# mjevans26/Satellite_ComputerVision

Hardware: AMD Instinct MI355X
Metric: tiles/sec (train) 256x256x4 U-Net (higher is better)
Workload: dtype bf16; 1 GPU; U-Net 256x256x4 bfloat16 training, batch 64 per GPU (BASELINE configs[1]); global_batch=64, parallelism=dp1, loss=weighted_categorical_crossentropy, optimizer=adam(9e-4)

## Files before the change

### include/satcv.h

```cpp
#ifndef SATCV_H
#define SATCV_H
#include <stdint.h>
#ifdef __cplusplus
extern "C" {
#endif

typedef double satcv_stat_t;

enum { SATCV_OK = 0, SATCV_ERR_INVALID = -1, SATCV_ERR_HIP = -2, SATCV_ERR_UNSUPPORTED = -3 };
enum { SATCV_F32 = 0, SATCV_BF16 = 1,
       SATCV_FP8 = 2 ,
       SATCV_FP8X = 3 ,
       SATCV_F64 = 4  };
#define SATCV_STAT_ROWS 32

const char* satcv_version(void);
const char* satcv_last_error(void);
int satcv_device_info(int32_t* out4);

int satcv_ingest_nhwc(const float* src, void* dst, int64_t npix, int32_t c, int32_t cpad,
                      int32_t dtype, void* stream);
int satcv_ingest_nhwc_scaled(const float* src, void* dst, int64_t npix, int32_t c, int32_t cpad, float mul, int32_t dtype, void* stream);
int satcv_ingest_chw(const void* src, int32_t src_kind, float scale, void* dst, int32_t n,
                     int32_t c, int32_t h, int32_t w, int32_t cpad, int32_t dtype, void* stream);

int satcv_pack_weights(const float* src, void* dst_fwd, void* dst_dgrad, int32_t kh, int32_t kw,
                       int32_t cin, int32_t cout, int32_t cin_pad, int32_t transposed,
                       int32_t dtype, void* stream);
typedef struct { const float* src; void* dst; int32_t mode, taps, cin, cout, kpad, npad; } satcv_pack_job;
int64_t satcv_pack_job_items(const satcv_pack_job* job);
int satcv_pack_weights_batched(const satcv_pack_job* jobs_dev, const int64_t* prefix_dev, int32_t njobs, int64_t total_items, int32_t dtype,
                               void* stream);

typedef struct satcv_conv_desc {
  const void* x0;
  const void* x1;
  int32_t c0, c1;
  const float* in_scale;
  const float* in_shift;
  int32_t in_relu;
  const void* w;
  const float* bias;
  void* y;
  int32_t ldy;
  satcv_stat_t* stats;
  int32_t stats_ld;
  int32_t n, h, w_;
  int32_t cout;
  int32_t cout_pad;
  int32_t kh, kw, dil;
  int32_t mode_in;
  int32_t mode_out;
  int32_t f;
  int32_t cstat;
  int32_t out_relu;
  int32_t dtype;
  int32_t accumulate;
  int32_t stride, hin, win;
  const float* out_scale;
  void* pool_y; int32_t pool_ld, pool_f;
  const void* bst_y; const void* bst_y1; int32_t bst_ld, bst_ld1, bst_split;
  const float* bst_scale; const float* bst_shift; const float* bst_mean; const float* bst_rstd; int32_t bst_relu;
  int32_t tile_policy;
  int32_t pair_n, pair_c0, pair_c1;
} satcv_conv_desc;
// ... 19 lines not shown
} satcv_wgrad_desc;
int64_t satcv_conv2d_wgrad_workspace(const satcv_wgrad_desc* d);
int satcv_conv2d_wgrad(const satcv_wgrad_desc* d, void* stream);

typedef struct satcv_reduce_job {
  const float* ws; float* dw;
  int32_t nslab, taps, kpad, npad, cin, nvalid, transposed, accumulate, lanes, pad_;
} satcv_reduce_job;
int satcv_conv2d_wgrad_reduce_job(const satcv_wgrad_desc* d, satcv_reduce_job* job);
int64_t satcv_reduce_job_items(const satcv_reduce_job* job);
int satcv_reduce_slabs_batched(const satcv_reduce_job* jobs_dev, const int64_t* prefix_dev, int32_t njobs, int64_t total_items, void* stream);

typedef struct satcv_bwdf_desc {
  const void* g; const void* yraw; int32_t ldg;
  const float* bn_scale; const float* bn_shift; const float* bn_mean; const float* bn_rstd;
  const float* bn_coef;
  int32_t linear;
  const void* x0; const void* x1; int32_t c0, c1;
  const float* in_scale; const float* in_shift; int32_t in_relu;
  const void* w_dgrad;
  void* dx; int32_t lddx;
  float* dw; int32_t cin, cout;
  int32_t n, h, w_;
  int32_t kh, kw, dil;
  float* workspace; int64_t workspace_bytes;
  int32_t dtype;
  int32_t accumulate;
  satcv_stat_t* bst_sums; int32_t bst_sums_ld;
  const float* bst_mean; const float* bst_rstd;
  int32_t bst_act_form;
  const void* dpool; int32_t lddp; const void* amax;
  const float* hg_dlogits; const float* hg_w; int32_t hg_ncls;
  int32_t defer_reduce;
} satcv_bwdf_desc;
int64_t satcv_conv2d_bwd_fused_workspace(const satcv_bwdf_desc* d);
int satcv_conv2d_bwd_fused(const satcv_bwdf_desc* d, void* stream);
int satcv_conv2d_bwd_fused_reduce_job(const satcv_bwdf_desc* d, satcv_reduce_job* job);

typedef struct satcv_ctbf_desc {
  const void* g; int32_t ldg;
  const void* yup; int32_t ldy;
  const float* bn_scale; const float* bn_shift; const float* bn_mean; const float* bn_rstd;
  const float* bn_c1; const float* bn_c2; int32_t linear;
  const void* x; int32_t ldx;
  const float* in_scale; const float* in_shift; int32_t in_relu;
  const void* w_dgrad; int32_t w_npad;
  void* dx; int32_t lddx;
  float* dw; int32_t cin, cout;
  int32_t n, h, w_, f;
  float* workspace; int64_t workspace_bytes;
  int32_t dtype, accumulate, defer_reduce;
  satcv_stat_t* bst_sums; int32_t bst_sums_ld; const float* bst_mean; const float* bst_rstd;
} satcv_ctbf_desc;
int64_t satcv_convt_bwd_fused_workspace(const satcv_ctbf_desc* d);
int satcv_convt_bwd_fused(const satcv_ctbf_desc* d, void* stream);
int satcv_convt_bwd_fused_reduce_job(const satcv_ctbf_desc* d, satcv_reduce_job* job);

int satcv_bn_finalize_train(satcv_stat_t* stats, int32_t stats_ld, int32_t c, float count,
                            const float* gamma, const float* beta, float eps, float momentum,
                            int32_t updates, int32_t bessel, float* moving_mean, float* moving_var,
                            float* scale, float* shift, float* mean, float* rstd, void* stream);
int satcv_bn_affine_infer(const float* gamma, const float* beta, const float* moving_mean,
                          const float* moving_var, float eps, int32_t c, float* scale, float* shift,
                          void* stream);
typedef struct satcv_bn_affine_job {
  const float* gamma; const float* beta; const float* moving_mean; const float* moving_var;
// ... 208 lines not shown
```

### satellite_computervision_amd/_lib.py

```python
import ctypes as C
import os

import torch

_HERE = os.path.dirname(os.path.abspath(__file__))
LIB_PATH = os.environ.get('SATCV_LIB') or os.path.join(_HERE, 'libsatcv.so')

F32, BF16, FP8, FP8X, F64 = 0, 1, 2, 3, 4
STAT_ROWS = 32
COMPOSITE_MAX_T = 256

c_i32, c_i64, c_f32, c_vp = C.c_int32, C.c_int64, C.c_float, C.c_void_p


class ConvDesc(C.Structure):
    _fields_ = [('x0', c_vp), ('x1', c_vp), ('c0', c_i32), ('c1', c_i32),
                ('in_scale', c_vp), ('in_shift', c_vp), ('in_relu', c_i32),
                ('w', c_vp), ('bias', c_vp), ('y', c_vp), ('ldy', c_i32),
                ('stats', c_vp), ('stats_ld', c_i32),
                ('n', c_i32), ('h', c_i32), ('w_', c_i32),
                ('cout', c_i32), ('cout_pad', c_i32),
                ('kh', c_i32), ('kw', c_i32), ('dil', c_i32),
                ('mode_in', c_i32), ('mode_out', c_i32), ('f', c_i32),
                ('cstat', c_i32), ('out_relu', c_i32), ('dtype', c_i32), ('accumulate', c_i32),
# ... 25 lines not shown
                ('crop_y', c_i32), ('crop_x', c_i32), ('crop_h', c_i32), ('crop_w', c_i32),
                ('origins', c_vp), ('total', c_i32), ('first', c_i32), ('dst', c_vp), ('dst_kind', c_i32),
                ('h', c_i32), ('w_', c_i32), ('ldd', c_i32), ('doff', c_i32), ('accumulate', c_i32)]


class CompositeDesc(C.Structure):
    _fields_ = [('src', c_vp), ('src_kind', c_i32), ('t', c_i32), ('c', c_i32), ('h', c_i32), ('w_', c_i32), ('offsets', c_vp),
                ('median', c_vp), ('ld_med', c_i32), ('coff_med', c_i32), ('norm', c_vp), ('ld_norm', c_i32), ('coff_norm', c_i32),
                ('use_fill', c_i32), ('fill', c_f32)]


class WgradDesc(C.Structure):
    _fields_ = [('x0', c_vp), ('x1', c_vp), ('c0', c_i32), ('c1', c_i32),
                ('in_scale', c_vp), ('in_shift', c_vp), ('in_relu', c_i32),
                ('dy', c_vp), ('lddy', c_i32), ('dw', c_vp),
                ('cin', c_i32), ('cout', c_i32),
                ('n', c_i32), ('h', c_i32), ('w_', c_i32),
                ('kh', c_i32), ('kw', c_i32), ('dil', c_i32),
                ('mode_dy', c_i32), ('f', c_i32), ('transposed', c_i32),
                ('workspace', c_vp), ('workspace_bytes', c_i64), ('dtype', c_i32), ('accumulate', c_i32), ('whole_chip', c_i32), ('defer_reduce', c_i32)]


class BwdfDesc(C.Structure):
    _fields_ = [('g', c_vp), ('yraw', c_vp), ('ldg', c_i32),
                ('bn_scale', c_vp), ('bn_shift', c_vp), ('bn_mean', c_vp), ('bn_rstd', c_vp), ('bn_coef', c_vp), ('linear', c_i32),
                ('x0', c_vp), ('x1', c_vp), ('c0', c_i32), ('c1', c_i32),
                ('in_scale', c_vp), ('in_shift', c_vp), ('in_relu', c_i32),
                ('w_dgrad', c_vp), ('dx', c_vp), ('lddx', c_i32),
                ('dw', c_vp), ('cin', c_i32), ('cout', c_i32),
                ('n', c_i32), ('h', c_i32), ('w_', c_i32), ('kh', c_i32), ('kw', c_i32), ('dil', c_i32),
                ('workspace', c_vp), ('workspace_bytes', c_i64), ('dtype', c_i32), ('accumulate', c_i32),
                ('bst_sums', c_vp), ('bst_sums_ld', c_i32), ('bst_mean', c_vp), ('bst_rstd', c_vp), ('bst_act_form', c_i32),
                ('dpool', c_vp), ('lddp', c_i32), ('amax', c_vp),
                ('hg_dlogits', c_vp), ('hg_w', c_vp), ('hg_ncls', c_i32), ('defer_reduce', c_i32)]


class CtbfDesc(C.Structure):
    _fields_ = [('g', c_vp), ('ldg', c_i32), ('yup', c_vp), ('ldy', c_i32),
                ('bn_scale', c_vp), ('bn_shift', c_vp), ('bn_mean', c_vp), ('bn_rstd', c_vp), ('bn_c1', c_vp), ('bn_c2', c_vp), ('linear', c_i32),
                ('x', c_vp), ('ldx', c_i32), ('in_scale', c_vp), ('in_shift', c_vp), ('in_relu', c_i32),
                ('w_dgrad', c_vp), ('w_npad', c_i32), ('dx', c_vp), ('lddx', c_i32), ('dw', c_vp), ('cin', c_i32), ('cout', c_i32),
                ('n', c_i32), ('h', c_i32), ('w_', c_i32), ('f', c_i32), ('workspace', c_vp), ('workspace_bytes', c_i64),
                ('dtype', c_i32), ('accumulate', c_i32), ('defer_reduce', c_i32),
                ('bst_sums', c_vp), ('bst_sums_ld', c_i32), ('bst_mean', c_vp), ('bst_rstd', c_vp)]


class ReduceJob(C.Structure):
    _fields_ = [('ws', c_vp), ('dw', c_vp), ('nslab', c_i32), ('taps', c_i32), ('kpad', c_i32), ('npad', c_i32), ('cin', c_i32), ('nvalid', c_i32),
                ('transposed', c_i32), ('accumulate', c_i32), ('lanes', c_i32), ('pad_', c_i32)]


class BnBwdDesc(C.Structure):
    _fields_ = [('da', c_vp), ('ldda', c_i32), ('dpool', c_vp), ('lddp', c_i32), ('f', c_i32),
                ('yraw', c_vp), ('ldy', c_i32),
                ('scale', c_vp), ('shift', c_vp), ('mean', c_vp), ('rstd', c_vp),
                ('sums', c_vp), ('sums_ld', c_i32), ('coef', c_vp),
                ('dy', c_vp), ('lddy_out', c_i32), ('dbias', c_vp),
                ('n', c_i32), ('h', c_i32), ('w_', c_i32), ('c', c_i32), ('dtype', c_i32), ('linear', c_i32),
                ('yraw1', c_vp), ('ldy1', c_i32), ('dy1', c_vp), ('lddy1', c_i32), ('c_split', c_i32),
                ('sk_sums', c_vp), ('sk_sums_ld', c_i32)]


class HeadDesc(C.Structure):
    _fields_ = [('x', c_vp), ('ldx', c_i32), ('cin', c_i32),
                ('in_scale', c_vp), ('in_shift', c_vp), ('w', c_vp), ('b', c_vp),
                ('ncls', c_i32), ('activation', c_i32), ('thresh', c_f32),
                ('probs', c_vp), ('classes', c_vp), ('dlogits', c_vp),
# ... 7 lines not shown
                ('c_out', c_vp), ('h_out', c_vp), ('ldh', c_i32), ('gates_out', c_vp),
                ('stats', c_vp), ('stats_ld', c_i32),
                ('dh_a', c_vp), ('lddh_a', c_i32), ('dh_b', c_vp), ('lddh_b', c_i32), ('dc_next', c_vp),
                ('dz_out', c_vp), ('lddz', c_i32), ('dc_prev_out', c_vp),
                ('npix', c_i64), ('filters', c_i32), ('rec_act', c_i32), ('act', c_i32), ('dtype', c_i32)]


class DenseSrc(C.Structure):
    _fields_ = [('x', c_vp), ('ld', c_i32), ('cin', c_i32), ('dtype', c_i32),
                ('in_scale', c_vp), ('in_shift', c_vp), ('in_relu', c_i32),
                ('hs', c_i32), ('ws', c_i32),
                ('dx', c_vp), ('lddx', c_i32), ('dx_dtype', c_i32)]


class DenseDesc(C.Structure):
    _fields_ = [('src', DenseSrc * 2), ('nsrc', c_i32),
                ('w', c_vp), ('b', c_vp), ('cout', c_i32),
                ('activation', c_i32), ('max_value', c_f32),
                ('out', c_vp), ('classes', c_vp), ('z_out', c_vp),
                ('npix', c_i64), ('h', c_i32), ('w_', c_i32),
                ('dout', c_vp), ('dz_out', c_vp), ('dw', c_vp), ('db', c_vp)]


_SIGS = {
    'satcv_version': (C.c_char_p, []),
    'satcv_last_error': (C.c_char_p, []),
    'satcv_device_info': (C.c_int, [C.POINTER(c_i32)]),
    'satcv_ingest_nhwc': (C.c_int, [c_vp, c_vp, c_i64, c_i32, c_i32, c_i32, c_vp]),
    'satcv_ingest_nhwc_scaled': (C.c_int, [c_vp, c_vp, c_i64, c_i32, c_i32, c_f32, c_i32, c_vp]),
    'satcv_ingest_chw': (C.c_int, [c_vp, c_i32, c_f32, c_vp, c_i32, c_i32, c_i32, c_i32, c_i32, c_i32, c_vp]),
    'satcv_pack_weights': (C.c_int, [c_vp, c_vp, c_vp, c_i32, c_i32, c_i32, c_i32, c_i32, c_i32, c_i32, c_vp]),
    'satcv_pack_job_items': (c_i64, [C.POINTER(PackJob)]),
    'satcv_pack_weights_batched': (C.c_int, [c_vp, c_vp, c_i32, c_i64, c_i32, c_vp]),
    'satcv_conv2d_igemm': (C.c_int, [C.POINTER(ConvDesc), c_vp]),
    'satcv_conv2d_igemm_pipelined': (C.c_int, [C.POINTER(ConvDesc)]),
    'satcv_conv2d_wgrad_workspace': (c_i64, [C.POINTER(WgradDesc)]),
    'satcv_conv2d_wgrad': (C.c_int, [C.POINTER(WgradDesc), c_vp]),
    'satcv_conv2d_wgrad_reduce_job': (C.c_int, [C.POINTER(WgradDesc), C.POINTER(ReduceJob)]),
    'satcv_reduce_job_items': (c_i64, [C.POINTER(ReduceJob)]),
    'satcv_reduce_slabs_batched': (C.c_int, [c_vp, c_vp, c_i32, c_i64, c_vp]),
    'satcv_conv2d_bwd_fused_workspace': (c_i64, [C.POINTER(BwdfDesc)]),
    'satcv_conv2d_bwd_fused': (C.c_int, [C.POINTER(BwdfDesc), c_vp]),
    'satcv_conv2d_bwd_fused_reduce_job': (C.c_int, [C.POINTER(BwdfDesc), C.POINTER(ReduceJob)]),
    'satcv_convt_bwd_fused_workspace': (c_i64, [C.POINTER(CtbfDesc)]),
    'satcv_convt_bwd_fused': (C.c_int, [C.POINTER(CtbfDesc), c_vp]),
    'satcv_convt_bwd_fused_reduce_job': (C.c_int, [C.POINTER(CtbfDesc), C.POINTER(ReduceJob)]),
    'satcv_bn_finalize_train': (C.c_int, [c_vp, c_i32, c_i32, c_f32, c_vp, c_vp, c_f32, c_f32, c_i32, c_i32,
                                          c_vp, c_vp, c_vp, c_vp, c_vp, c_vp, c_vp]),
    'satcv_bn_affine_infer': (C.c_int, [c_vp, c_vp, c_vp, c_vp, c_f32, c_i32, c_vp, c_vp, c_vp]),
    'satcv_bn_affine_infer_batched': (C.c_int, [c_vp, c_i32, c_f32, c_vp]),
    'satcv_bn_relu_pool': (C.c_int, [c_vp, c_vp, c_vp, c_vp, c_i32, c_vp, c_vp, c_i32, c_i32, c_i32, c_i32, c_i32, c_i32, c_i32, c_vp]),
    'satcv_bn_relu_pool_amax': (C.c_int, [c_vp, c_vp, c_vp, c_vp, c_i32, c_vp, c_vp, c_vp, c_i32, c_i32, c_i32, c_i32, c_i32, c_i32, c_i32, c_vp]),
    'satcv_bn_bwd_reduce': (C.c_int, [C.POINTER(BnBwdDesc), c_vp]),
    'satcv_bn_bwd_finalize': (C.c_int, [c_vp, c_i32, c_i32, c_f32, c_vp, c_vp, c_vp, c_i32, c_vp]),
    'satcv_bn_bwd_apply': (C.c_int, [C.POINTER(BnBwdDesc), c_vp]),
    'satcv_bn_bwd_finalize2': (C.c_int, [c_vp, c_i32, c_vp, c_i32, c_i32, c_f32, c_vp, c_vp, c_vp, c_vp, c_vp, c_vp, c_vp, c_i32, c_vp]),
    'satcv_maxpool': (C.c_int, [c_vp, c_vp, c_i32, c_i32, c_i32, c_i32, c_i32, c_i32, c_i32, c_i32, c_vp]),
    'satcv_affine_requant': (C.c_int, [c_vp, c_i32, c_vp, c_vp, c_i32, c_vp, c_i32, c_i64, c_i32, c_i32, c_i32, c_vp]),
    'satcv_add_act': (C.c_int, [c_vp, c_vp, c_vp, c_vp, c_vp, c_vp, c_i32, c_vp, c_i64, c_i32, c_i32, c_vp]),
    'satcv_relu_bwd': (C.c_int, [c_vp, c_vp, c_i64, c_i32, c_vp]),
    'satcv_bias_grad_workspace': (c_i64, [c_i64, c_i32]),
    'satcv_bias_grad': (C.c_int, [c_vp, c_i32, c_i64, c_i32, c_i32, c_vp, c_vp, c_vp]),
    'satcv_upsample_head': (C.c_int, [c_vp, c_i32, c_i32, c_i32, c_i32, c_i32, c_i32, c_f32, c_vp, c_vp, c_vp]),
    'satcv_dropout_mask': (C.c_int, [C.c_uint64, C.c_uint64, c_f32, c_i64, c_vp, c_vp]),
    'satcv_dropout_apply': (C.c_int, [c_vp, c_i32, c_vp, c_vp, c_i32, c_vp, c_i32, c_i32, c_vp, c_i32, c_i32, c_i32, c_i32, c_i32, c_vp]),
    'satcv_tile_channel_mean': (C.c_int, [C.POINTER(TileDesc), c_vp, c_vp]),
# ... 71 lines not shown
```

### satellite_computervision_amd/csrc/api.hip

```cpp
#include "common.hpp"
#include <cstring>
#include <cstdarg>
#include <cstdio>
#include <cstdlib>
#include <mutex>
#include <vector>

static thread_local char g_err[512] = "";
void satcv_set_error(const char* fmt, ...) {
  va_list ap;
  va_start(ap, fmt);
  vsnprintf(g_err, sizeof(g_err), fmt, ap);
  va_end(ap);
}

extern "C" const char* satcv_version(void) { return "satcv 0.1 (gfx950)"; }
extern "C" const char* satcv_last_error(void) { return g_err; }

extern "C" int satcv_device_info(int32_t* out4) {
  SATCV_CHECK(out4, "device_info: null");
  int dev = 0;
  SATCV_HIP(hipGetDevice(&dev));
  hipDeviceProp_t p;
  SATCV_HIP(hipGetDeviceProperties(&p, dev));
// ... 74 lines not shown
extern "C" int satcv_prof_enable(int32_t kind_mask) {
  g_prof_mask = kind_mask;
  return SATCV_OK;
}
extern "C" int satcv_prof_collect(int32_t kind, double* total_ms, int64_t* launches, double* flops) {
  SATCV_CHECK(kind >= 0 && kind < PROF_KINDS && total_ms && launches && flops, "prof_collect: bad args");
  std::lock_guard<std::mutex> lk(g_prof_mu);
  double ms = 0, fl = 0;
  for (auto& r : g_prof[kind]) {
    (void)hipEventSynchronize(r.b);
    float t = 0;
    if (hipEventElapsedTime(&t, r.a, r.b) == hipSuccess) ms += t;
    fl += r.flops;
    (void)hipEventDestroy(r.a); (void)hipEventDestroy(r.b);
  }
  *total_ms = ms; *launches = (int64_t)g_prof[kind].size(); *flops = fl;
  g_prof[kind].clear();
  return SATCV_OK;
}

static int env_int(const char* name, int dflt) { const char* e = getenv(name); return e ? atoi(e) : dflt; }
int g_opt_igemm_db = env_int("SATCV_DB", 1);
int g_opt_wgrad_db = env_int("SATCV_WGRAD_DB", 1);
int g_opt_igemm_sched = env_int("SATCV_IGEMM_SCHED", 0);
int g_opt_igemm_thin = env_int("SATCV_THIN", 1);
int g_opt_igemm_m16 = env_int("SATCV_M16", 1);
int g_opt_m16p = env_int("SATCV_M16P", 1);
extern int g_m16p_launches;
int g_tr_launches = 0;
int g_opt_thin_roles = env_int("SATCV_THIN_ROLES", 1);
int g_opt_m16p_prio = env_int("SATCV_M16P_PRIO", 30);
int g_opt_wgrad_m16 = env_int("SATCV_WGRAD_M16", 0);
int g_opt_splitk = env_int("SATCV_SPLITK", 0);
static int* opt_slot(const char* key) {
  if (!key) return nullptr;
  if (!strcmp(key, "igemm_db")) return &g_opt_igemm_db;
  if (!strcmp(key, "igemm_thin")) return &g_opt_igemm_thin;
  if (!strcmp(key, "wgrad_db")) return &g_opt_wgrad_db;
  if (!strcmp(key, "igemm_sched")) return &g_opt_igemm_sched;
  if (!strcmp(key, "splitk")) return &g_opt_splitk;
  if (!strcmp(key, "igemm_m16")) return &g_opt_igemm_m16;
  if (!strcmp(key, "thin_roles")) return &g_opt_thin_roles;
  if (!strcmp(key, "thin_roles_launches")) return &g_tr_launches;
  if (!strcmp(key, "m16p")) return &g_opt_m16p;
  if (!strcmp(key, "m16p_prio")) return &g_opt_m16p_prio;
  if (!strcmp(key, "wgrad_m16")) return &g_opt_wgrad_m16;
  if (!strcmp(key, "m16p_launches")) return &g_m16p_launches;
  return nullptr;
}
extern "C" int satcv_set_option(const char* key, int32_t value) {
  int* p = opt_slot(key);
  SATCV_CHECK(p, "set_option: unknown key '%s'", key ? key : "(null)");
  *p = value;
  return SATCV_OK;
}
extern int g_ws_launches;
extern "C" int satcv_get_option(const char* key, int32_t* value) {
  if (key && value && !strcmp(key, "igemm_thin_launches")) { *value = g_ws_launches; return SATCV_OK; }
  int* p = opt_slot(key);
  SATCV_CHECK(p && value, "get_option: unknown key '%s'", key ? key : "(null)");
  *value = *p;
  return SATCV_OK;
}

static uint32_t g_crc_tab[8][256];
static bool g_crc_init = [] {
  for (uint32_t i = 0; i < 256; ++i) {
    uint32_t c = i;
    for (int k = 0; k < 8; ++k) c = (c & 1) ? (c >> 1) ^ 0x82F63B78u : c >> 1;
    g_crc_tab[0][i] = c;
  }
  for (uint32_t i = 0; i < 256; ++i)
    for (int t = 1; t < 8; ++t) g_crc_tab[t][i] = (g_crc_tab[t - 1][i] >> 8) ^ g_crc_tab[0][g_crc_tab[t - 1][i] & 0xff];
  return true;
}();
extern "C" uint32_t satcv_crc32c(const void* data, uint64_t nbytes, uint32_t crc_in) {
  const unsigned char* p = reinterpret_cast<const unsigned char*>(data);
  uint32_t c = ~crc_in;
  while (nbytes >= 8) {
    uint32_t lo, hi;
// ... 10 lines not shown
```

### satellite_computervision_amd/csrc/common.hpp

```cpp
#pragma once
#include <hip/hip_runtime.h>
#include <hip/hip_fp8.h>
#include <stdint.h>
#include <type_traits>
#include "../../include/satcv.h"

typedef __bf16 bf16;
typedef __hip_fp8_e4m3 fp8;
struct fp8s : public __hip_fp8_e4m3 { using __hip_fp8_e4m3::__hip_fp8_e4m3; };
using i32x8 = __attribute__((ext_vector_type(8))) int;
using i32x4 = __attribute__((ext_vector_type(4))) int;

template <typename T> struct KTraits { static constexpr int EL = 8, SUB = 1; };
template <> struct KTraits<fp8s> { static constexpr int EL = 16, SUB = 2; };
using bf16x8 = __attribute__((ext_vector_type(8))) __bf16;
using bf16x4 = __attribute__((ext_vector_type(4))) __bf16;
using short4v = __attribute__((ext_vector_type(4))) short;
using f32x16 = __attribute__((ext_vector_type(16))) float;
using f32x4 = __attribute__((ext_vector_type(4))) float;

void satcv_set_error(const char* fmt, ...);
#define SATCV_CHECK(cond, ...)                        \
  do {                                                \
    if (!(cond)) {                                    \
// ... 196 lines not shown
    const bf16x8 v = __builtin_bit_cast(bf16x8, r.q[0]);
#pragma unroll
    for (int i = 0; i < 8; ++i) out[i] = (float)v[i];
  } else if constexpr (std::is_same<T, float>::value) {
    const float* f = reinterpret_cast<const float*>(&r.q[0]);
#pragma unroll
    for (int i = 0; i < 8; ++i) out[i] = f[i];
  } else {
    const fp8* b = reinterpret_cast<const fp8*>(&r.q);
#pragma unroll
    for (int i = 0; i < 8; ++i) out[i] = (float)b[i];
  }
}
template <typename T>
__device__ __forceinline__ void keep8(const Raw8<T>& r) {
  if constexpr (std::is_same<T, fp8>::value) { asm volatile("" :: "v"(r.q.x), "v"(r.q.y)); }
  else {
#pragma unroll
    for (int i = 0; i < Raw8<T>::NQ; ++i) asm volatile("" :: "v"(r.q[i].x), "v"(r.q[i].y), "v"(r.q[i].z), "v"(r.q[i].w));
  }
}
template <typename T>
__device__ __forceinline__ Raw8<T> select8(bool keep, const Raw8<T>& r) {
  Raw8<T> o;
  if constexpr (std::is_same<T, fp8>::value) {
    o.q = make_uint2(keep ? r.q.x : 0u, keep ? r.q.y : 0u);
  } else {
#pragma unroll
    for (int i = 0; i < Raw8<T>::NQ; ++i) o.q[i] = make_uint4(keep ? r.q[i].x : 0u, keep ? r.q[i].y : 0u, keep ? r.q[i].z : 0u, keep ? r.q[i].w : 0u);
  }
  return o;
}

template <typename T>
__device__ __forceinline__ float round_to(float x) {
  if constexpr (std::is_same<T, bf16>::value) return (float)(bf16)x;
  else if constexpr (std::is_same<T, fp8>::value) return (float)(fp8)x;
  else return x;
}

__device__ __forceinline__ float wave_sum(float v) {
#pragma unroll
  for (int o = 32; o > 0; o >>= 1) v += __shfl_xor(v, o, 64);
  return v;
}

typedef __attribute__((address_space(3))) char satcv_lds_char;
__device__ __forceinline__ unsigned lds_addr_of(const void* p) { return (unsigned)(uintptr_t)(satcv_lds_char*)p; }
__device__ __forceinline__ void lds_dma16(const void* gbase, unsigned voff, unsigned lds_dst) {
  unsigned keep;
  asm volatile("s_mov_b32 %0, m0\n\ts_mov_b32 m0, %3\n\ts_nop 0\n\tglobal_load_lds_dwordx4 %2, %1\n\ts_mov_b32 m0, %0"
               : "=&s"(keep) : "s"(gbase), "v"(voff), "s"(lds_dst) : "memory");
}
__device__ __forceinline__ void dma_wait_all() { asm volatile("s_waitcnt vmcnt(0)" ::: "memory"); }

#define SATCV_STAT_REPL 32
```

### satellite_computervision_amd/csrc/conv_bwd_fused.hip

```cpp
#include "igemm_common.hpp"
#include <cstdlib>
#include <cstring>

#ifndef BWDF_ABL
#define BWDF_ABL 0
#endif
#define FABL(bit) ((BWDF_ABL & (bit)) != 0)

int wgrad_reduce_slabs(const float* ws, float* dw, int nslab, int taps, int kpad, int npad, int cin, int nvalid, int accumulate, hipStream_t st);
void reduce_job_fill(satcv_reduce_job* job, const float* ws, float* dw, int nslab, int taps, int kpad, int npad, int cin, int nvalid, int transposed, int accumulate);
void satcv_prof_begin(int kind, double flops, hipStream_t st);
void satcv_prof_end(int kind, hipStream_t st);

struct BwdfArgs {
  IgemmArgs e;
  const void* g; const void* yraw; int ldg;
  const float* bn_scale; const float* bn_shift; const float* bn_mean; const float* bn_rstd; const float* bn_coef; int bn_c, linear;
  const void* x0; const void* x1; int c0, c1;
  const float* in_scale; const float* in_shift; int in_relu;
  const void* w;
  float* ws;
  int tiles_x, tiles_y;
  satcv_stat_t* bst_sums; int bst_ld; const float* bst_mean; const float* bst_rstd;
  int bst_act_form;
  const void* dp; int lddp; const unsigned char* amax;
  const float* hg_dl; const float* hg_w;
};

__device__ __forceinline__ bf16x4 tr_read4(const bf16* p) {
  short4v v = __builtin_amdgcn_ds_read_tr16_b64_v4i16((__attribute__((address_space(3))) short4v*)(p));
  return __builtin_bit_cast(bf16x4, v);
}

template <int CIN, int COUT, int NW, int WPS, bool POOL = false, bool NODG = false, int CINS = CIN, bool HG = false>
__global__ __launch_bounds__(NW * 64, WPS) void bwd_fused_kernel(const BwdfArgs a, const int total_tiles) {
  static_assert(!HG || !POOL, "the head feeds a decoder block");
  typedef bf16 T;
  constexpr int TW = 32, TH = 8, BM = 256, RL = TH + 2, CL = TW + 2, PITCH = CL, EL = 8, NTHREADS = NW * 64;
  constexpr int SD = COUT / 8, SX = CIN / 8, SXR = CINS / 8;
  constexpr int DSTRIDE = RL * PITCH * EL;
  constexpr int XSTRIDE = BM * EL + 32;
  static_assert((DSTRIDE * 2) % 256 == 64 && (XSTRIDE * 2) % 256 == 64, "plane strides must be 64 B modulo 256 B");
  constexpr int D_ITEMS = RL * CL * SD, DI = (D_ITEMS + NTHREADS - 1) / NTHREADS;
  constexpr int X_ITEMS = BM * SXR, XI = X_ITEMS / NTHREADS;
  static_assert(X_ITEMS % NTHREADS == 0 && NTHREADS % SD == 0 && NTHREADS % SXR == 0, "item -> thread mapping");
  constexpr int XPIX_STEP = NTHREADS / SXR;
  static_assert(XPIX_STEP % 32 == 0, "x items of a thread must share a column");
  constexpr int MT = 8 / NW, NT = CIN / 32;
#ifdef BWDF_NOBAL
  constexpr int NTILE = (CIN / 32) * (COUT / 32) * 9, FULL = (NTILE + NW - 1) / NW, REM = 0, WT = FULL;
#else
  constexpr int NTILE = (CIN / 32) * (COUT / 32) * 9, FULL = NTILE / NW, REM = NTILE % NW, WT = FULL + (REM ? 1 : 0);
#endif
  constexpr bool GUARD = FULL * NW > NTILE;
  constexpr int WPP = REM ? NW / REM : 1, KPW = REM ? 16 / WPP : 0;
  static_assert(REM == 0 || (NW % REM == 0 && 16 % WPP == 0 && KPW % 2 == 0), "left-over products must split evenly along K");
  constexpr int W_ITEMS = NODG ? 0 : 9 * SD * CIN;
  constexpr size_t R0_BYTES = ((size_t)(SD * DSTRIDE + SX * XSTRIDE) * sizeof(T) + 127) / 128 * 128;
  constexpr size_t W_BYTES = (size_t)W_ITEMS * EL * sizeof(T);
  constexpr size_t O_BYTES = (size_t)BM * (CIN + 8) * sizeof(T);
  constexpr bool O_ALIAS = O_BYTES <= (size_t)SD * DSTRIDE * sizeof(T);
  constexpr size_t TAB_BYTES = (size_t)(SD * 32 + SX * 16 + (HG ? 2 * COUT : 0)) * sizeof(float);
  static_assert(!NODG || O_ALIAS || true, "");
  constexpr size_t O_OFF = O_ALIAS ? 0 : (R0_BYTES + W_BYTES + TAB_BYTES + 127) / 128 * 128;
  extern __shared__ __attribute__((aligned(16))) unsigned char smem_raw[];
  T* ldsD = reinterpret_cast<T*>(smem_raw);
  T* ldsX = ldsD + SD * DSTRIDE;
  T* ldsW = reinterpret_cast<T*>(smem_raw + R0_BYTES);
  float* tabD = reinterpret_cast<float*>(smem_raw + R0_BYTES + W_BYTES);
// ... 12 lines not shown
    const float sc = a.bn_scale[ch], sh = a.bn_shift[ch], mu = a.bn_mean[ch], rs = a.bn_rstd[ch], c1 = a.bn_coef[ch], c2 = a.bn_coef[a.bn_c + ch];
    float* t = tabD + (ch >> 3) * 32 + (ch & 7);
    t[0] = sc; t[8] = sh; t[16] = -sc * c2 * rs; t[24] = sc * (c2 * rs * mu - c1);
  }
  if constexpr (HG) {
    for (int ch = tid; ch < COUT; ch += NTHREADS) {
      float* t = tabH + (ch >> 3) * 16 + (ch & 7);
      t[0] = a.hg_w[ch * 2]; t[8] = a.hg_w[ch * 2 + 1];
    }
  }
  for (int ch = tid; ch < CINS; ch += NTHREADS) {
    float* t = tabX + (ch >> 3) * 16 + (ch & 7);
    t[0] = a.in_scale ? a.in_scale[ch] : 1.f; t[8] = a.in_scale ? a.in_shift[ch] : 0.f;
  }
  const float lin_lo = a.linear ? -INFINITY : 0.f;
  const bool xaff = a.in_scale != nullptr;
  const unsigned xrelu_lim = a.in_relu != 0 ? 0u : 0x80008000u;

  const int slot_d = tid % SD, slot_x = tid % SXR;
  constexpr int DPK = (DI + 2) / 3;
  unsigned d_pk[DPK];
#pragma unroll
  for (int k = 0; k < DPK; ++k) d_pk[k] = 0;
#pragma unroll
  for (int j = 0; j < DI; ++j) {
    const int it = tid + j * NTHREADS;
    const int p = it / SD, c = p % CL, L = p / CL;
    d_pk[j / 3] |= (unsigned)(it < D_ITEMS ? (L << 6) | c : 0x3ff) << (10 * (j % 3));
  }
  auto d_item = [&](int j) -> int { return (int)((d_pk[j / 3] >> (10 * (j % 3))) & 0x3ffu); };
  const int g_rowstride = a.e.w_ * a.ldg;
  const unsigned gy_lane = (unsigned)slot_d * EL;
  const int xch0 = slot_x * EL;
  const bool xsecond = xch0 >= a.c0;
  const T* xsrc = xsecond ? reinterpret_cast<const T*>(a.x1) + (xch0 - a.c0) : reinterpret_cast<const T*>(a.x0) + xch0;
  const int xcs = xsecond ? a.c1 : a.c0;
  const int xq0 = tid / SXR;
  const int x_l0 = slot_x * XSTRIDE + xq0 * EL;
  const int x_eoff0 = ((xq0 / TW) * a.e.w_ + (xq0 % TW)) * xcs, x_estep = (XPIX_STEP / TW) * a.e.w_ * xcs;

  int a_off[MT];
#pragma unroll
  for (int m = 0; m < MT; ++m) {
    const int q = (wave * MT + m) * 32 + r;
    a_off[m] = ((q / TW) * PITCH + (q % TW)) * EL;
  }
  const int gi = lane >> 4, i16 = lane & 15;
  const int chb = 16 * (gi & 1) + 4 * (i16 & 3);
  const int pk = 8 * (gi >> 1) + (i16 >> 2);
  const int tr_x = (chb >> 3) * XSTRIDE + pk * EL + (chb & 7);
  const int tr_d = (chb >> 3) * DSTRIDE + pk * EL + (chb & 7);

  auto tile_origin = [&](int v, int& n0, int& y0, int& x0) {
    const int tx = v % a.tiles_x; v /= a.tiles_x;
    const int ty = v % a.tiles_y;
    n0 = v / a.tiles_y; y0 = ty * TH; x0 = tx * TW;
  };
  auto next_origin = [&](int& n0, int& y0, int& x0) {
    x0 += TW;
    if (x0 >= a.e.w_) { x0 = 0; y0 += TH; if (y0 >= a.e.h) { y0 = 0; ++n0; } }
  };
  Raw8<T> rg[HG ? 1 : DI], ry[DI], rx[XI];
  float2 rdl[HG ? DI : 1];
  Raw8<T> rp[POOL ? DI : 1];
  uint2 ra[POOL ? DI : 1];
  const int hp = a.e.h >> 1, wpool = a.e.w_ >> 1;
  unsigned valid = 0;
  auto issue_loads = [&](int n0, int y0, int x0) -> unsigned {
    unsigned vm = 0;
// ... 110 lines not shown
          }
        }
        Raw8<T> v;
        if constexpr (FABL(2) && !HG) { v = rg[j]; v.q[0].x ^= ry[j].q[0].x; }
        else {
          bf16x8 o;
#pragma unroll
          for (int e = 0; e < 8; ++e) {
            const float act = yv[e] * prm[e] + prm[8 + e];
            const float gm = act > lin_lo ? gv[e] : 0.f;
            o[e] = (bf16)(prm[e] * gm + (prm[16 + e] * yv[e] + prm[24 + e]));
          }
          v.q[0] = __builtin_bit_cast(uint4, o);
        }
        v = select8<T>((valid >> j) & 1u, v);
        const int pk_ = d_item(j);
        if (pk_ != 0x3ff) lstore8<T>(ldsD + slot_d * DSTRIDE + __mul24((pk_ >> 6) * CL + (pk_ & 63), EL), v);
        __builtin_amdgcn_sched_barrier(0);
      }
    }
    {
      float sc[8], sh[8];
      if (xaff) {
        int toff = slot_x * 16;
        asm volatile("" : "+v"(toff));
        const float4* tp = reinterpret_cast<const float4*>(tabX + toff);
        const float4 s0 = tp[0], s1 = tp[1], h0 = tp[2], h1 = tp[3];
        sc[0] = s0.x; sc[1] = s0.y; sc[2] = s0.z; sc[3] = s0.w; sc[4] = s1.x; sc[5] = s1.y; sc[6] = s1.z; sc[7] = s1.w;
        sh[0] = h0.x; sh[1] = h0.y; sh[2] = h0.z; sh[3] = h0.w; sh[4] = h1.x; sh[5] = h1.y; sh[6] = h1.z; sh[7] = h1.w;
      }
#pragma unroll
      for (int j = 0; j < XI; ++j) {
        Raw8<T> v = rx[j];
        if (xaff) v = affine8_lim(v, sc, sh, xrelu_lim);
        lstore8<T>(ldsX + x_l0 + j * (XPIX_STEP * EL), v);
      }
    }
    __syncthreads();
    const int tn0 = n0, ty0 = y0, tx0 = x0;
    if (t + 1 < t_hi) { next_origin(n0, y0, x0); valid = issue_loads(n0, y0, x0); }

#pragma unroll
    for (int tt = 0; tt < FULL; ++tt) {
      if (!FABL(8) && (!GUARD || tt < FULL - 1 || __builtin_amdgcn_readfirstlane(wave) + (FULL - 1) * NW < NTILE)) {
        const T* xa = ldsX + w_xo[tt] + tr_x;
        const T* da = ldsD + w_do[tt] + tr_d;
        bf16x4 fa[2][2], fb[2][2];
        auto read_k = [&](const T* xp, const T* dp, int u, int buf) {
          const int xq = u * 16 * EL, dq = ((u >> 1) * PITCH + (u & 1) * 16) * EL;
          fa[buf][0] = tr_read4(xp + xq); fa[buf][1] = tr_read4(xp + xq + 4 * EL);
          fb[buf][0] = tr_read4(dp + dq); fb[buf][1] = tr_read4(dp + dq + 4 * EL);
        };
        read_k(xa, da, 0, 0);
#pragma unroll 1
        for (int grp = 0; grp < TH / 2; ++grp) {
          const T* xp = xa + grp * (64 * EL);
          const T* dp = da + grp * (2 * PITCH * EL);
          const int wrap = grp + 1 < TH / 2 ? 1 : 1 - TH / 2;
#pragma unroll
          for (int u = 0; u < 4; ++u) {
            asm volatile("" ::: "memory");
            if (u < 3) read_k(xp, dp, u + 1, (u + 1) & 1);
            else read_k(xp + wrap * (64 * EL), dp + wrap * (2 * PITCH * EL), 0, 0);
            __builtin_amdgcn_sched_barrier(0);
            const bf16x8 afr = __builtin_shufflevector(fa[u & 1][0], fa[u & 1][1], 0, 1, 2, 3, 4, 5, 6, 7);
            const bf16x8 bfr = __builtin_shufflevector(fb[u & 1][0], fb[u & 1][1], 0, 1, 2, 3, 4, 5, 6, 7);
// ... 148 lines not shown
      atomicAdd(rowp + a.bst_ld + tid, (satcv_stat_t)s2);
    }
  }
}

template <int CIN, int COUT, int NW, bool NODG = false>
struct BwdfGeom {
  static constexpr int SD = COUT / 8, SX = CIN / 8;
  static constexpr size_t R0 = ((size_t)(SD * (10 * 34 * 8) + SX * (256 * 8 + 32)) * 2 + 127) / 128 * 128;
  static constexpr size_t O_BYTES = (size_t)256 * (CIN + 8) * 2;
  static constexpr bool O_ALIAS = O_BYTES <= (size_t)SD * (10 * 34 * 8) * 2;
  static constexpr size_t BASE = R0 + (NODG ? 0 : (size_t)9 * SD * CIN * 16) + (size_t)(SD * 32 + SX * 16 + 2 * COUT) * 4;
  static constexpr size_t LDS0 = O_ALIAS ? BASE : (BASE + 127) / 128 * 128 + O_BYTES;
  static constexpr size_t RED = (size_t)16 * NW * 64 * 4;
  static constexpr size_t LDS = LDS0 > RED ? LDS0 : RED;
};

static int g_ncu = 0;
static int bwdf_grid(size_t lds, int waves, int wps, long long total) {
  if (!g_ncu) {
    int dev = 0; hipDeviceProp_t p;
    if (hipGetDevice(&dev) != hipSuccess || hipGetDeviceProperties(&p, dev) != hipSuccess) return -1;
    g_ncu = p.multiProcessorCount;
  }
  int per_cu = (int)((160 * 1024) / lds);
  const int by_waves = 4 * wps / waves;
  if (per_cu > by_waves) per_cu = by_waves;
  if (per_cu < 1) per_cu = 1;
  long long grid = (long long)g_ncu * per_cu;
  if (grid > total) grid = total;
  return (int)grid;
}

static bool bwdf_shape_ok(const satcv_bwdf_desc* d, int& cin_s) {
  cin_s = d->c0 + d->c1;
  if (d->dtype != SATCV_BF16 || d->kh != 3 || d->kw != 3 || d->dil != 1) return false;
  if (d->x1 && d->c0 % 8 != 0) return false;
  if (d->h % 8 != 0 || d->w_ % 32 != 0) return false;
  if (d->ldg % 8 != 0 || ((uintptr_t)d->g % 16) != 0 || ((uintptr_t)d->yraw % 16) != 0) return false;
  if (d->hg_dlogits && (!d->hg_w || d->hg_ncls != 2 || d->dpool || ((uintptr_t)d->hg_dlogits % 8) != 0)) return false;
  if (d->dx && (d->lddx % 8 != 0 || ((uintptr_t)d->dx % 16) != 0)) return false;
  if ((long long)d->w_ * d->ldg >= (1 << 23)) return false;
  if (d->dpool) {
    if (!d->amax || d->lddp % 8 != 0 || ((uintptr_t)d->dpool % 16) != 0 || ((uintptr_t)d->amax % 8) != 0 || d->x1) return false;
    if (d->dx) return cin_s == 32 && d->cin == 32 && d->cout == 64;
    return cin_s == 16 && d->cin <= 16 && d->cout == 32 && !d->bst_sums;
  }
  if (!d->dx) return false;
  if (d->bst_sums && cin_s == 64 && d->cout == 64) return false;
  if (!((cin_s == 32 && d->cout == 32) || (cin_s == 64 && d->cout == 32) || (cin_s == 64 && d->cout == 64))) return false;
  if (d->cin != cin_s) return false;
  return true;
}

template <int CIN, int COUT, int NW, int WPS, bool POOL = false, bool NODG = false, int CINS = CIN, bool HG = false>
static int bwdf_launch(const satcv_bwdf_desc* d, hipStream_t st, bool query, int64_t* ws_bytes, satcv_reduce_job* job = nullptr) {
  using G = BwdfGeom<CIN, COUT, NW, NODG>;
  static_assert(G::LDS <= 160 * 1024, "tile + weights exceed the LDS");
  const long long total = (long long)d->n * (d->h / 8) * (d->w_ / 32);
  const int grid = bwdf_grid(G::LDS, NW, WPS, total);
  if (grid <= 0) { satcv_set_error("bwd_fused: device query failed"); return SATCV_ERR_HIP; }
  const size_t need = (size_t)grid * 9 * CIN * COUT * sizeof(float);
  if (job) { reduce_job_fill(job, d->workspace, d->dw, grid, 9, CIN, COUT, d->cin, COUT, 0, d->accumulate); return SATCV_OK; }
  if (query) { *ws_bytes = (int64_t)need; return SATCV_OK; }
  SATCV_CHECK((size_t)d->workspace_bytes >= need, "bwd_fused: workspace %lld < %zu", (long long)d->workspace_bytes, need);
  BwdfArgs a;
  memset(&a, 0, sizeof(a));
  a.e.y = d->dx; a.e.ldy = d->lddx; a.e.n = d->n; a.e.h = d->h; a.e.w_ = d->w_; a.e.cout = CIN; a.e.cout_pad = CIN; a.e.cstat = CIN;
  a.e.imgs = 1; a.e.rpi = 8; a.e.tiles_x = d->w_ / 32; a.e.tiles_y = d->h / 8; a.e.n_tiles = 1;
  a.g = d->g; a.yraw = d->yraw; a.ldg = d->ldg;
  a.bn_scale = d->bn_scale; a.bn_shift = d->bn_shift; a.bn_mean = d->bn_mean; a.bn_rstd = d->bn_rstd; a.bn_coef = d->bn_coef; a.bn_c = d->cout; a.linear = d->linear;
  a.x0 = d->x0; a.x1 = d->x1; a.c0 = d->c0; a.c1 = d->c1; a.in_scale = d->in_scale; a.in_shift = d->in_shift; a.in_relu = d->in_relu;
  a.w = d->w_dgrad; a.ws = d->workspace; a.tiles_x = d->w_ / 32; a.tiles_y = d->h / 8;
  a.bst_sums = d->bst_sums; a.bst_ld = d->bst_sums_ld; a.bst_mean = d->bst_mean; a.bst_rstd = d->bst_rstd; a.bst_act_form = d->bst_act_form;
  a.dp = d->dpool; a.lddp = d->lddp; a.amax = reinterpret_cast<const unsigned char*>(d->amax);
  a.hg_dl = d->hg_dlogits; a.hg_w = d->hg_w;
  auto kern = bwd_fused_kernel<CIN, COUT, NW, WPS, POOL, NODG, CINS, HG>;
  { const int rc = satcv_ensure_dynamic_lds(reinterpret_cast<const void*>(kern), G::LDS); if (rc) return rc; }
  const double flops = (NODG ? 2.0 : 4.0) * d->n * d->h * d->w_ * (double)CINS * COUT * 9;
  satcv_prof_begin(3, flops, st);
  hipLaunchKernelGGL(kern, dim3(grid), dim3(NW * 64), G::LDS, st, a, (int)total);
  satcv_prof_end(3, st);
  hipError_t e = hipGetLastError();
  if (e != hipSuccess) { satcv_set_error("bwd_fused launch: %s", hipGetErrorString(e)); return SATCV_ERR_HIP; }
  if (d->defer_reduce) return SATCV_OK;
  return wgrad_reduce_slabs(d->workspace, d->dw, grid, 9, CIN, COUT, d->cin, COUT, d->accumulate, st);
}

static int bwdf_dispatch(const satcv_bwdf_desc* d, hipStream_t st, bool query, int64_t* ws_bytes, satcv_reduce_job* job = nullptr) {
  int cin_s;
  if (!bwdf_shape_ok(d, cin_s)) return SATCV_ERR_UNSUPPORTED;
  if (d->dpool) {
    if (d->dx) return bwdf_launch<32, 64, 4, 1, true, false>(d, st, query, ws_bytes, job);
    return bwdf_launch<32, 32, 8, 2, true, true, 16>(d, st, query, ws_bytes, job);
  }
  if (cin_s == 32 && d->hg_dlogits) return bwdf_launch<32, 32, 8, 2, false, false, 32, true>(d, st, query, ws_bytes, job);
  if (d->hg_dlogits) return SATCV_ERR_UNSUPPORTED;
  if (cin_s == 32) return bwdf_launch<32, 32, 8, 2>(d, st, query, ws_bytes, job);
  if (d->cout == 32) return bwdf_launch<64, 32, 8, 2>(d, st, query, ws_bytes, job);
  return bwdf_launch<64, 64, 4, 1>(d, st, query, ws_bytes, job);
}

extern "C" int satcv_conv2d_bwd_fused_reduce_job(const satcv_bwdf_desc* d, satcv_reduce_job* job) {
  SATCV_CHECK(d && job && d->dw && d->workspace, "bwd_fused_reduce_job: null pointer");
  return bwdf_dispatch(d, nullptr, false, nullptr, job);
}

extern "C" int64_t satcv_conv2d_bwd_fused_workspace(const satcv_bwdf_desc* d) {
  int64_t nb = -1;
  if (!d || bwdf_dispatch(d, nullptr, true, &nb) != SATCV_OK) return -1;
  return nb;
}

extern "C" int satcv_conv2d_bwd_fused(const satcv_bwdf_desc* d, void* stream) {
  SATCV_CHECK(d && (d->g || d->hg_dlogits) && d->yraw && d->x0 && d->dw && d->workspace && (d->dx == nullptr || d->w_dgrad), "bwd_fused: null pointer");
  SATCV_CHECK(d->bn_scale && d->bn_shift && d->bn_mean && d->bn_rstd && d->bn_coef, "bwd_fused: BatchNorm coefficients missing");
  SATCV_CHECK((d->c1 == 0) == (d->x1 == nullptr) && d->n > 0 && d->h > 0 && d->w_ > 0, "bwd_fused: bad dims");
  SATCV_CHECK(!d->bst_sums || (d->bst_sums_ld >= d->c0 + d->c1 && (d->bst_act_form ? d->in_scale == nullptr
                               : (d->in_scale && d->in_shift && d->in_relu && d->bst_mean && d->bst_rstd))),
              "bwd_fused: the fused sums need the input's BatchNorm (in_scale / in_shift with ReLU, bst_mean / bst_rstd), or an activated input with bst_act_form");
  const int rc = bwdf_dispatch(d, reinterpret_cast<hipStream_t>(stream), false, nullptr);
  if (rc == SATCV_ERR_UNSUPPORTED) satcv_set_error("bwd_fused: shape outside the kernel's limits (ask satcv_conv2d_bwd_fused_workspace first)");
  return rc;
}
```

### satellite_computervision_amd/csrc/conv_igemm.hip

```cpp
#include "igemm_common.hpp"
#include <cstdlib>

template <typename T, int TW, int WM, int WN, int MT, int NT, int KS>
__global__ __launch_bounds__(WM* WN * 64) void igemm_kernel(const IgemmArgs a) {
  constexpr int NTHREADS = WM * WN * 64;
  constexpr int BM = WM * MT * 32;
  constexpr int BN = WN * NT * 32;
  constexpr int TH = BM / TW;
  constexpr int KC = KS * 16;
  constexpr int SLOTS = KC / 8;
  extern __shared__ __attribute__((aligned(16))) unsigned char smem_raw[];
  T* ldsA = reinterpret_cast<T*>(smem_raw);
  const int a_elems = SLOTS * a.rl * a.pitch * 8;
  T* ldsB = ldsA + a_elems;

  const int tid = threadIdx.x;
  const int lane = tid & 63;
  const int wave = tid >> 6;
  const int wm = wave / WN, wn = wave % WN;
  const int r = lane & 31, hh = lane >> 5;

  int bid = blockIdx.x;
  const int nt = bid % a.n_tiles;
  int mt = bid / a.n_tiles;
// ... 208 lines not shown
template <typename T, int TW>
static int launch_tw(IgemmArgs& a, hipStream_t st) {
  const int cin = a.c0 + a.c1;
  const int nspace = a.mode_out ? a.cstat : a.cout;
  const bool ks2 = (cin % 32 == 0) && (!a.x1 || a.c0 % 32 == 0) && (a.mode_in != 1 || a.c0 % 32 == 0) &&
                   (a.kh * a.kw == 1);
  int rc = SATCV_ERR_UNSUPPORTED;
  if (nspace >= 128 && nspace % 128 == 0)
    rc = ks2 ? launch_cfg<T, TW, 2, 2, 2, 2, 2>(a, st) : launch_cfg<T, TW, 2, 2, 2, 2, 1>(a, st);
  if (rc == SATCV_ERR_UNSUPPORTED && nspace >= 64 && nspace % 64 == 0)
    rc = ks2 ? launch_cfg<T, TW, 2, 2, 2, 1, 2>(a, st) : launch_cfg<T, TW, 2, 2, 2, 1, 1>(a, st);
  if (rc == SATCV_ERR_UNSUPPORTED)
    rc = ks2 ? launch_cfg<T, TW, 4, 1, 2, 1, 2>(a, st) : launch_cfg<T, TW, 4, 1, 2, 1, 1>(a, st);
  if (rc == SATCV_ERR_UNSUPPORTED)
    rc = launch_cfg<T, TW, 2, 1, 2, 1, 1>(a, st);
  if (rc == SATCV_ERR_UNSUPPORTED) satcv_set_error("igemm: no tile configuration fits the LDS for this shape");
  return rc;
}

template <typename T>
static int launch_t(IgemmArgs& a, hipStream_t st) {
  switch (igemm_pick_tw(a.w_)) {
    case 32: return launch_tw<T, 32>(a, st);
    case 16: return launch_tw<T, 16>(a, st);
    default: return launch_tw<T, 8>(a, st);
  }
}

void satcv_prof_begin(int kind, double flops, hipStream_t st);
void satcv_prof_end(int kind, hipStream_t st);

static int igemm_fill_args(const satcv_conv_desc* d, IgemmArgs& a) {
  SATCV_CHECK(d && d->x0 && d->w && d->y, "igemm: null pointer");
  SATCV_CHECK(d->c0 > 0 && d->c0 % 16 == 0 && d->c1 % 16 == 0, "igemm: channels must be multiples of 16 (c0=%d c1=%d)", d->c0, d->c1);
  SATCV_CHECK(d->dtype != SATCV_FP8X || (d->c0 % 64 == 0 && d->c1 % 64 == 0 && !d->in_scale), "igemm: the scaled fp8 path needs channels %% 64 == 0 and no input transform");
  SATCV_CHECK((d->c1 == 0) == (d->x1 == nullptr), "igemm: x1/c1 mismatch");
  SATCV_CHECK(d->kh >= 1 && d->kw >= 1 && (d->kh & 1) && (d->kw & 1) && d->dil >= 1, "igemm: bad taps");
  SATCV_CHECK(d->n > 0 && d->h > 0 && d->w_ > 0 && d->cout > 0, "igemm: bad dims");
  SATCV_CHECK(satcv_pixels_ok(d->n, d->h, d->w_, d->f) && d->cout <= (1 << 20) && d->c0 <= (1 << 20) && d->c1 <= (1 << 20) &&
              d->kh <= 15 && d->kw <= 15 && d->dil <= (1 << 15) && d->f <= 16 && d->stride <= 16,
              "igemm: extents out of range (n*h*w must stay below 2^31 pixels, channels below 2^20)");
  SATCV_CHECK(d->cstat > 0, "igemm: cstat");
  SATCV_CHECK((!d->mode_in && !d->mode_out) || (d->f >= 2 && d->kh == 1 && d->kw == 1), "igemm: s2d/d2s need 1x1 taps and f>=2");
  SATCV_CHECK(!(d->accumulate && d->stats), "igemm: accumulate with statistics");
  SATCV_CHECK(!(d->mode_in && d->in_scale), "igemm: s2d source cannot carry an input transform");
  a.x0 = d->x0; a.x1 = d->x1; a.c0 = d->c0; a.c1 = d->c1;
  a.in_scale = d->in_scale; a.in_shift = d->in_shift; a.in_relu = d->in_relu;
  a.w = d->w; a.bias = d->bias; a.out_scale = d->out_scale; a.y = d->y; a.ldy = d->ldy;
  a.pool_y = d->pool_y; a.pool_ld = d->pool_ld; a.pool_f = d->pool_f;
  SATCV_CHECK(!d->pool_y || (d->pool_f >= 2 && !d->mode_out && !d->accumulate && d->h % d->pool_f == 0 && d->w_ % d->pool_f == 0 && d->pool_ld >= d->cout &&
                             d->cout % (d->dtype == SATCV_F32 ? 4 : (d->dtype == SATCV_BF16 ? 8 : 16)) == 0),
              "igemm: fused max-pool needs pool_f >= 2 dividing h and w_, plain output mode, whole 16-byte channel vectors");
  a.stats = d->stats; a.stats_ld = d->stats_ld;
  a.n = d->n; a.h = d->h; a.w_ = d->w_;
  a.hs = d->mode_in ? d->h * d->f : d->h; a.ws = d->mode_in ? d->w_ * d->f : d->w_;
  a.cout = d->cout; a.cout_pad = d->cout_pad;
  a.kh = d->kh; a.kw = d->kw; a.dil = d->dil;
  a.mode_in = d->mode_in; a.mode_out = d->mode_out; a.f = d->f;
  a.cstat = d->cstat; a.out_relu = d->out_relu; a.accumulate = d->accumulate;
  a.stride = d->stride > 1 ? d->stride : 1;
  if (a.stride > 1) {
    SATCV_CHECK(!d->mode_in && !d->mode_out && d->hin > 0 && d->win > 0 && d->h == (d->hin - 1) / a.stride + 1 && d->w_ == (d->win - 1) / a.stride + 1,
                "igemm: strided conv needs hin/win with h=(hin-1)/stride+1");
    a.hs = d->hin; a.ws = d->win;
  }
  a.dbg = 0;
  a.ksplit = 1; a.kslab = nullptr;
  a.bst_y = d->bst_y; a.bst_y1 = d->bst_y1; a.bst_ld = d->bst_ld; a.bst_ld1 = d->bst_ld1; a.bst_split = d->bst_y1 ? d->bst_split : 0;
  a.bst_scale = d->bst_scale; a.bst_shift = d->bst_shift; a.bst_mean = d->bst_mean; a.bst_rstd = d->bst_rstd; a.bst_relu = d->bst_relu;
  a.tile_policy = d->tile_policy;
  a.pair_n = d->pair_n; a.pair_c0 = d->pair_c0; a.pair_c1 = d->pair_c1;
  if (d->pair_n || d->pair_c0 || d->pair_c1) {
    const int epv = d->dtype == SATCV_F32 ? 4 : (d->dtype == SATCV_BF16 ? 8 : 16);
    SATCV_CHECK(d->pair_n > 0 && d->n == 2 * d->pair_n, "igemm: pair store needs n == 2 * pair_n (n=%d pair_n=%d)", d->n, d->pair_n);
    SATCV_CHECK(!d->mode_out && !d->accumulate && !d->stats && !d->bst_y, "igemm: pair store needs a plain store (no mode_out / accumulate / stats / bst_y)");
    SATCV_CHECK(d->pair_c0 >= 0 && d->pair_c1 >= 0 && d->pair_c0 + d->cout <= d->ldy && d->pair_c1 + d->cout <= d->ldy,
                "igemm: pair channel offsets %d / %d + cout %d exceed ldy %d", d->pair_c0, d->pair_c1, d->cout, d->ldy);
    SATCV_CHECK(d->pair_c0 % epv == 0 && d->pair_c1 % epv == 0, "igemm: pair channel offsets must be multiples of %d", epv);
  }
  if (d->bst_y) {
    SATCV_CHECK(d->stats && d->bst_scale && d->bst_shift && d->bst_mean && d->bst_rstd, "igemm: bst_y needs stats and the four BatchNorm vectors");
    SATCV_CHECK(!d->accumulate && !d->mode_out && !d->out_relu && !d->pool_y && d->cstat == d->cout, "igemm: bst_y needs a plain, non-accumulating store");
    SATCV_CHECK(d->bst_ld >= (d->bst_y1 ? d->bst_split : d->cout) && (!d->bst_y1 || (d->bst_split > 0 && d->bst_split < d->cout && d->bst_ld1 >= d->cout - d->bst_split)),
                "igemm: bst_y channel strides");
  }
  if (a.mode_in == 1) {
    SATCV_CHECK(!d->x1, "igemm: s2d with dual source");
    a.c1 = a.c0 * (d->f * d->f - 1);
  }
  return SATCV_OK;
}

static bool igemm_force_generic() {
  static const bool v = [] { const char* e = getenv("SATCV_IGEMM"); return e && e[0] == 'g'; }();
  return v;
}

extern "C" int satcv_conv2d_igemm_pipelined(const satcv_conv_desc* d) {
  IgemmArgs a;
  if (!d || igemm_fill_args(d, a) != SATCV_OK || igemm_force_generic()) return 0;
  if (a.kh == 3 && a.kw == 3 && a.stride == 1 && a.dil >= a.h && a.dil >= a.w_) { a.kh = a.kw = 1; a.dil = 1; }
  if (d->bst_y && a.dil == 3) {
    IgemmArgs b = a;
    b.bst_y = nullptr; b.bst_y1 = nullptr;
    if (igemm_ws_launch(b, d->dtype, nullptr, true) == SATCV_OK) return 0;
  }
  return igemm_fast_launch(a, d->dtype, nullptr, true) == SATCV_OK ? 1 : 0;
}

extern "C" int satcv_conv2d_igemm(const satcv_conv_desc* d, void* stream) {
  IgemmArgs a;
  int rc = igemm_fill_args(d, a);
  if (rc) return rc;
  hipStream_t st = reinterpret_cast<hipStream_t>(stream);
  const double flops = 2.0 * d->n * d->h * d->w_ * (double)d->cout * (double)(a.c0 + a.c1) * d->kh * d->kw;
  if (a.kh == 3 && a.kw == 3 && a.stride == 1 && a.dil >= a.h && a.dil >= a.w_) {
    const size_t esz = d->dtype == SATCV_BF16 ? 2 : 4;
    a.w = reinterpret_cast<const unsigned char*>(a.w) + (size_t)4 * ((a.c0 + a.c1) / 8) * a.cout_pad * 8 * esz;
    a.kh = a.kw = 1; a.dil = 1;
  }
  satcv_prof_begin(d->kh * d->kw > 1 ? 0 : 1, flops, st);
  rc = SATCV_ERR_UNSUPPORTED;
  if (!igemm_force_generic()) {
    rc = convt_thin_launch(a, d->dtype, st);
    if (rc == SATCV_ERR_UNSUPPORTED) rc = convt_thin_dgrad_launch(a, d->dtype, st);
    if (rc == SATCV_ERR_UNSUPPORTED) rc = igemm_tr_launch(a, d->dtype, st, false);
    if (rc == SATCV_ERR_UNSUPPORTED) rc = igemm_ws_launch(a, d->dtype, st, false);
    if (rc == SATCV_ERR_UNSUPPORTED) rc = igemm_fast_launch(a, d->dtype, st);
  }
  if (rc != SATCV_ERR_UNSUPPORTED) {  }
  else if (d->dtype == SATCV_FP8 || d->dtype == SATCV_FP8X) { satcv_set_error("igemm: this fp8 shape is outside the pipelined kernel's limits"); rc = SATCV_ERR_UNSUPPORTED; }
  else if (d->out_scale || d->pool_y || d->bst_y || d->pair_n) { satcv_set_error("igemm: out_scale / pool_y / bst_y / pair store need the pipelined kernel"); rc = SATCV_ERR_UNSUPPORTED; }
  else if (d->dtype == SATCV_BF16) rc = launch_t<bf16>(a, st);
  else if (d->dtype == SATCV_F32) rc = launch_t<float>(a, st);
  else { satcv_set_error("igemm: bad dtype %d", d->dtype); rc = SATCV_ERR_INVALID; }
  satcv_prof_end(d->kh * d->kw > 1 ? 0 : 1, st);
  return rc;
}
```

### satellite_computervision_amd/csrc/conv_igemm_ws.hip

```cpp
#include "igemm_common.hpp"
#include <cstdlib>
extern int g_opt_igemm_thin;
int g_ws_launches = 0;

#ifndef SATCV_ABLATE
#define SATCV_ABLATE 0
#endif
#define WABL(bit) ((SATCV_ABLATE & (bit)) != 0)
#ifdef SATCV_STAMP
__device__ unsigned long long g_stamp_ws[8][8][8];
extern "C" int satcv_debug_read_stamps_ws(unsigned long long* out) { return hipMemcpyFromSymbol(out, HIP_SYMBOL(g_stamp_ws), sizeof(g_stamp_ws)) == hipSuccess ? 0 : -1; }
#define STAMP(t) do { __builtin_amdgcn_sched_barrier(0); asm volatile("s_memtime %0\n\ts_waitcnt lgkmcnt(0)" : "=s"(t) :: "memory"); __builtin_amdgcn_sched_barrier(0); } while (0)
#define STAMP_V(t) do { __builtin_amdgcn_sched_barrier(0); asm volatile("s_waitcnt vmcnt(0)\n\ts_memtime %0\n\ts_waitcnt lgkmcnt(0)" : "=s"(t) :: "memory"); __builtin_amdgcn_sched_barrier(0); } while (0)
#endif

template <typename T, int CIN, int NT, int WPS, int WN = 1, int DIL = 1>
__global__ __launch_bounds__(256 * WN, WPS) void igemm_ws_kernel(const IgemmArgs a, const int total_tiles) {
  constexpr int TW = 32, TH = 8, WM = 4, MT = 2, BM = 256, BN = WN * NT * 32, NTHREADS = 256 * WN, EL = 8;
  constexpr int SLOTS = CIN / EL, CL = TW + 2 * DIL, PITCH = CL, RL = TH + 2 * DIL;
  constexpr int PLANE = RL * PITCH * EL;
  constexpr int WANT = (SLOTS >= 8 ? 16 : 128 / SLOTS) / (int)sizeof(T), BANKSPAN = 128 / (int)sizeof(T);
  constexpr int SPAD = ((WANT - PLANE % BANKSPAN) % BANKSPAN + BANKSPAN) % BANKSPAN;
  constexpr int SLOT_STRIDE = PLANE + SPAD;
  constexpr int A_ITEMS = RL * CL * SLOTS, AI = (A_ITEMS + NTHREADS - 1) / NTHREADS;
  constexpr int W_ITEMS = 9 * SLOTS * BN;
  constexpr int OPITCH = BN + 16 / (int)sizeof(T);
  constexpr size_t A_BYTES = (size_t)SLOTS * SLOT_STRIDE * sizeof(T);
  constexpr size_t O_BYTES = (size_t)BM * OPITCH * sizeof(T) + (size_t)(WM + 1) * 2 * BN * sizeof(float);
  constexpr size_t R0_BYTES = ((A_BYTES > O_BYTES ? A_BYTES : O_BYTES) + 127) / 128 * 128;
  extern __shared__ __attribute__((aligned(16))) unsigned char smem_raw[];
  T* ldsA = reinterpret_cast<T*>(smem_raw);
  T* ldsW = reinterpret_cast<T*>(smem_raw + R0_BYTES);

  const int tid = threadIdx.x, lane = tid & 63, wave = tid >> 6;
  const int wm = wave / WN, wn = wave % WN;
  const int r = lane & 31, hh = lane >> 5;
  const int slot_t = tid % SLOTS;
  const T* wp = reinterpret_cast<const T*>(a.w);

  for (int it = tid; it < W_ITEMS; it += NTHREADS) {
    const int co = it % BN, run = it / BN;
    const Raw8<T> v = gload8<T>(wp + ((size_t)run * a.cout_pad + co) * EL);
    lstore8<T>(ldsW + (size_t)it * EL, v);
  }
  const int ch0 = slot_t * EL;
  const bool second = ch0 >= a.c0;
  const T* src = second ? reinterpret_cast<const T*>(a.x1) + (ch0 - a.c0) : reinterpret_cast<const T*>(a.x0) + ch0;
  const int cs = second ? a.c1 : a.c0;
  float sc[8], sh[8];
#pragma unroll
  for (int e = 0; e < 8; ++e) { sc[e] = a.in_scale ? a.in_scale[ch0 + e] : 1.f; sh[e] = a.in_scale ? a.in_shift[ch0 + e] : 0.f; }
  const bool aff = a.in_scale != nullptr;
  const unsigned relu_lim = a.in_relu != 0 ? 0u : 0x80008000u;

  int a_l[AI], a_yx[AI], a_eoff[AI];
#pragma unroll
  for (int j = 0; j < AI; ++j) {
    const int it = tid + j * NTHREADS;
    const int pix = it / SLOTS, c = pix % CL, L = pix / CL;
    a_l[j] = it < A_ITEMS ? slot_t * SLOT_STRIDE + (L * PITCH + c) * EL : -1;
    a_yx[j] = ((L - DIL) << 16) | ((c - DIL) & 0xffff);
    a_eoff[j] = ((L - DIL) * a.w_ + (c - DIL)) * cs;
  }
  int a_off[MT];
#pragma unroll
  for (int m = 0; m < MT; ++m) {
    const int q = (wm * MT + m) * 32 + r;
    a_off[m] = ((q / TW) * PITCH + (q % TW)) * EL;
  }

  auto tile_origin = [&](int v, int& n0, int& y0, int& x0) {
    const int tx = v % a.tiles_x; v /= a.tiles_x;
    const int ty = v % a.tiles_y;
    n0 = v / a.tiles_y; y0 = ty * TH; x0 = tx * TW;
  };
  auto next_origin = [&](int& n0, int& y0, int& x0) {
    x0 += TW;
    if (x0 >= a.w_) { x0 = 0; y0 += TH; if (y0 >= a.h) { y0 = 0; ++n0; } }
  };
  Raw8<T> ra[AI];
  unsigned valid = 0;
  auto issue_loads = [&](int n0, int y0, int x0) -> unsigned {
    unsigned vm = 0;
    const int ylo = -y0, yhi = a.h - y0, xlo = -x0, xhi = a.w_ - x0;
    const T* base = src + ((size_t)(n0 * a.h + y0) * a.w_ + x0) * cs;
#pragma unroll
    for (int j = 0; j < AI; ++j) {
      const int dy = a_yx[j] >> 16, dx = (int)(short)(a_yx[j] & 0xffff);
      const bool ok = a_l[j] >= 0 && dy >= ylo && dy < yhi && dx >= xlo && dx < xhi;
      vm |= (ok ? 1u : 0u) << j;
      int off = ok ? a_eoff[j] : 0;
      asm volatile("" : "+v"(off));
      if (!WABL(4)) ra[j] = gload8<T>(base + off);
      else ra[j] = zero8<T>();
    }
    return vm;
  };

  const int G = gridDim.x;
  const int xcd = blockIdx.x & 7, nx = G >> 3, remx = G & 7;
  const int bid = (xcd < remx ? xcd * (nx + 1) : remx * (nx + 1) + (xcd - remx) * nx) + (blockIdx.x >> 3);
  const int per = total_tiles / G, extra = total_tiles % G;
  const int t_lo = bid * per + (bid < extra ? bid : extra), t_hi = t_lo + per + (bid < extra ? 1 : 0);

  double carry[2] = {0.0, 0.0};
  int n0, y0, x0;
  if (t_lo < t_hi) { tile_origin(t_lo, n0, y0, x0); valid = issue_loads(n0, y0, x0); }
  __syncthreads();
#ifdef SATCV_STAMP
  unsigned long long q0, q1, q2, q3, q4, q5, q6, q7, q8, z[8] = {0, 0, 0, 0, 0, 0, 0, 0};
#endif
  for (int t = t_lo; t < t_hi; ++t) {
#ifdef SATCV_STAMP
    STAMP(q0);
    STAMP_V(q1);
#endif
#pragma unroll
    for (int j = 0; j < AI; ++j) {
      Raw8<T> v = ra[j];
      if (aff) { if constexpr (std::is_same<T, bf16>::value) v = affine8_lim(v, sc, sh, relu_lim); else v = affine8<T>(v, sc, sh, a.in_relu); }
      v = select8<T>((valid >> j) & 1u, v);
      if (a_l[j] >= 0) lstore8<T>(ldsA + a_l[j], v);
    }
#ifdef SATCV_STAMP
    STAMP(q2);
#endif
    __syncthreads();
#ifdef SATCV_STAMP
    STAMP(q3);
#endif
    const int tn0 = n0, ty0 = y0, tx0 = x0;
    if (t + 1 < t_hi) { next_origin(n0, y0, x0); valid = issue_loads(n0, y0, x0); }
#ifdef SATCV_STAMP
    STAMP(q4);
#endif
    f32x16 acc[MT][NT];
#pragma unroll
    for (int m = 0; m < MT; ++m)
#pragma unroll
      for (int n = 0; n < NT; ++n)
#pragma unroll
        for (int i = 0; i < 16; ++i) acc[m][n][i] = 0.f;
    {
      constexpr int KS = CIN / 16, STEPS = 9 * KS;
      FragT<T> af[2][MT], bf[2][NT];
      auto read_step = [&](int st, int buf) {
        const int tap = st / KS, ks = st % KS;
        const int tap_off = ((tap / 3) * DIL * PITCH + (tap % 3) * DIL) * EL;
        const int slot = ks * 2 + hh;
#pragma unroll
        for (int m = 0; m < MT; ++m) af[buf][m] = lds_frag<T>(ldsA + slot * SLOT_STRIDE + a_off[m] + tap_off);
#pragma unroll
// ... 9 lines not shown
        for (int m = 0; m < MT; ++m)
#pragma unroll
          for (int n = 0; n < NT; ++n) { if (!WABL(2)) mma32<T>(acc[m][n], af[st & 1][m], bf[st & 1][n]); }
      }
    }
#ifdef SATCV_STAMP
    STAMP(q5);
#endif
    __syncthreads();
#ifdef SATCV_STAMP
    STAMP(q6);
#endif
    igemm_epilogue<T, TW, WM, WN, MT, NT, WABL(1), true, false, false, DIL == 1>(a, acc, tn0, ty0, tx0, 0, smem_raw, carry);
#ifdef SATCV_STAMP
    STAMP(q7);
#endif
    __syncthreads();
#ifdef SATCV_STAMP
    STAMP(q8);
    z[0] += q1 - q0; z[1] += q2 - q1; z[2] += q3 - q2; z[3] += q4 - q3; z[4] += q5 - q4; z[5] += q6 - q5; z[6] += q7 - q6; z[7] += q8 - q7;
#endif
  }
  if (a.stats && tid < BN && tid < a.cout && t_lo < t_hi) {
    satcv_stat_t* rowp = a.stats + (size_t)(blockIdx.x % SATCV_STAT_ROWS) * 2 * a.stats_ld;
    atomicAdd(rowp + tid, (satcv_stat_t)carry[0]);
    atomicAdd(rowp + a.stats_ld + tid, (satcv_stat_t)carry[1]);
  }
#ifdef SATCV_STAMP
  if (blockIdx.x < 8 && lane == 0)
    for (int i = 0; i < 8; ++i) g_stamp_ws[blockIdx.x][wave][i] = z[i] / (unsigned long long)max(t_hi - t_lo, 1);
#endif
}

template <typename T, int CIN, int NT, int WPS, int WN = 1, int DIL = 1>
static int ws_cfg(IgemmArgs& a, hipStream_t st, bool dry) {
  constexpr int TW = 32, TH = 8, BN = WN * NT * 32, SLOTS = CIN / 8, RL = TH + 2 * DIL, PITCH = TW + 2 * DIL;
  constexpr int ES = (int)sizeof(T);
  constexpr int PLANE = RL * PITCH * 8;
  constexpr int WANT = (SLOTS >= 8 ? 16 : 128 / SLOTS) / ES, BANKSPAN = 128 / ES;
  constexpr int SPAD = ((WANT - PLANE % BANKSPAN) % BANKSPAN + BANKSPAN) % BANKSPAN;
  constexpr size_t A_BYTES = (size_t)SLOTS * (PLANE + SPAD) * ES;
  constexpr size_t O_BYTES = (size_t)256 * (BN + 16 / ES) * ES + (size_t)5 * 2 * BN * 4;
  constexpr size_t R0 = ((A_BYTES > O_BYTES ? A_BYTES : O_BYTES) + 127) / 128 * 128;
  constexpr size_t LDS = R0 + (size_t)9 * SLOTS * BN * 8 * ES;
  static_assert(LDS <= 160 * 1024, "weights + tile exceed the LDS");
  a.halh = a.halw = DIL;
  a.tiles_x = cdiv(a.w_, TW); a.tiles_y = cdiv(a.h, TH);
  a.rpi = TH; a.imgs = 1; a.ngroups = a.n; a.seg = RL; a.rl = RL; a.cl = PITCH; a.pitch = PITCH; a.n_tiles = 1;
  const long long total = (long long)a.n * a.tiles_y * a.tiles_x;
  if (total <= 0 || total > 0x7fffffffLL) return SATCV_ERR_UNSUPPORTED;
  if (dry) return SATCV_OK;
  auto kern = igemm_ws_kernel<T, CIN, NT, WPS, WN, DIL>;
  { const int rc = satcv_ensure_dynamic_lds(reinterpret_cast<const void*>(kern), LDS); if (rc) return rc; }
  static int ncu = 0;
  if (!ncu) {
    int dev = 0; hipDeviceProp_t p;
    if (hipGetDevice(&dev) != hipSuccess || hipGetDeviceProperties(&p, dev) != hipSuccess) { satcv_set_error("ws: device query failed"); return SATCV_ERR_HIP; }
    ncu = p.multiProcessorCount;
  }
  int per_cu = (int)((160 * 1024) / LDS);
  if (per_cu > WPS) per_cu = WPS;
  if (per_cu < 1) per_cu = 1;
  long long grid = (long long)ncu * per_cu;
  if (grid > total) grid = total;
  hipLaunchKernelGGL(kern, dim3((unsigned)grid), dim3(256 * WN), LDS, st, a, (int)total);
  ++g_ws_launches;
  hipError_t e = hipGetLastError();
  if (e != hipSuccess) { satcv_set_error("igemm_ws launch: %s", hipGetErrorString(e)); return SATCV_ERR_HIP; }
  return SATCV_OK;
}

int igemm_ws_launch(IgemmArgs& a, int dtype, hipStream_t st, bool dry) {
  if (!g_opt_igemm_thin || (dtype != SATCV_BF16 && dtype != SATCV_FP8)) return SATCV_ERR_UNSUPPORTED;
  const int cin = a.c0 + a.c1;
  if (a.kh != 3 || a.kw != 3 || (a.dil != 1 && a.dil != 3) || a.stride != 1 || a.mode_in || a.mode_out || a.bst_y) return SATCV_ERR_UNSUPPORTED;
  if (a.accumulate && (a.accumulate != 1 || dtype != SATCV_BF16 || a.stats || a.pool_y || a.out_relu || a.out_scale)) return SATCV_ERR_UNSUPPORTED;
  if (a.pool_y && (8 % a.pool_f != 0 || 32 % a.pool_f != 0)) return SATCV_ERR_UNSUPPORTED;
  if (a.dil == 3) {
    if (dtype != SATCV_BF16 || a.pool_y || a.pair_n || !(cin == 16 || cin == 32) || !(a.cout == 16 || a.cout == 32) || a.cout_pad != 32 || a.cstat != a.cout) return SATCV_ERR_UNSUPPORTED;
    if (a.x1 && (a.c0 % 8 != 0)) return SATCV_ERR_UNSUPPORTED;
    if (a.h % 8 != 0 || a.w_ % 32 != 0 || a.ldy % 8 != 0 || ((uintptr_t)a.y % 16) != 0) return SATCV_ERR_UNSUPPORTED;
    return cin == 16 ? ws_cfg<bf16, 16, 1, 2, 1, 3>(a, st, dry) : ws_cfg<bf16, 32, 1, 2, 1, 3>(a, st, dry);
  }
  if (a.cout == 16 && dtype == SATCV_BF16 && !a.pool_y && (cin == 16 || cin == 32) && a.cout_pad == 32 && a.cstat == 16 && !(a.x1 && (a.c0 % 8 != 0)) &&
      a.h % 8 == 0 && a.w_ % 32 == 0 && a.ldy % 8 == 0 && ((uintptr_t)a.y % 16) == 0) {
    return cin == 16 ? ws_cfg<bf16, 16, 1, 3>(a, st, dry) : ws_cfg<bf16, 32, 1, 3>(a, st, dry);
  }
  if (!(cin == 16 || cin == 32 || cin == 64) || !(a.cout == 32 || a.cout == 64) || a.cout_pad != a.cout || a.cstat != a.cout) return SATCV_ERR_UNSUPPORTED;
  if (a.x1 && (a.c0 % 8 != 0)) return SATCV_ERR_UNSUPPORTED;
  const int epv = dtype == SATCV_FP8 ? 16 : 8;
  if (a.h % 8 != 0 || a.w_ % 32 != 0 || a.ldy % epv != 0 || ((uintptr_t)a.y % 16) != 0) return SATCV_ERR_UNSUPPORTED;
  if (dtype == SATCV_FP8) {
    if (a.stats || cin == 16 || (a.pool_y && a.pool_ld % 16 != 0)) return SATCV_ERR_UNSUPPORTED;
    if (a.cout == 32) return cin == 32 ? ws_cfg<fp8, 32, 1, 3>(a, st, dry) : ws_cfg<fp8, 64, 1, 2>(a, st, dry);
    return cin == 32 ? ws_cfg<fp8, 32, 2, 2>(a, st, dry) : ws_cfg<fp8, 64, 1, 1, 2>(a, st, dry);
  }
  if (a.cout == 32) {
    if (cin == 16) return ws_cfg<bf16, 16, 1, 3>(a, st, dry);
    if (cin == 32) return ws_cfg<bf16, 32, 1, 3>(a, st, dry);
    return ws_cfg<bf16, 64, 1, 2>(a, st, dry);
  }
  if (cin == 16) return ws_cfg<bf16, 16, 2, 2>(a, st, dry);
  if (cin == 32) return ws_cfg<bf16, 32, 2, 2>(a, st, dry);
  return ws_cfg<bf16, 64, 1, 1, 2>(a, st, dry);
}
```

### satellite_computervision_amd/csrc/elementwise.hip

```cpp
#include "common.hpp"
#include <cstdlib>

#define EW_BLOCK 256
static inline int ew_grid(long long items, int cap = 0) {
  static const int dflt = [] { const char* e = getenv("SATCV_EW_PER_CU"); const int v = e ? atoi(e) : 6; return 256 * (v >= 1 ? v : 6); }();
  if (cap <= 0) cap = dflt;
  long long b = (items + EW_BLOCK - 1) / EW_BLOCK;
  if (b < 1) b = 1;
  if (b > cap) b = cap;
  return (int)b;
}
#define LAUNCH_OK(name)                                                          \
  do {                                                                           \
    hipError_t e__ = hipGetLastError();                                          \
    if (e__ != hipSuccess) {                                                     \
      satcv_set_error(name " launch: %s", hipGetErrorString(e__));               \
      return SATCV_ERR_HIP;                                                      \
    }                                                                            \
  } while (0)
#define DISPATCH_T(dtype, ...)                                                   \
  do {                                                                           \
    if ((dtype) == SATCV_BF16) { using T = bf16; __VA_ARGS__; }                  \
    else if ((dtype) == SATCV_F32) { using T = float; __VA_ARGS__; }             \
    else { satcv_set_error("bad dtype %d", (int)(dtype)); return SATCV_ERR_INVALID; } \
// ... 65 lines not shown
static inline int rup(int a, int b) { return (a + b - 1) / b * b; }

template <typename T, int EL = 8>
__global__ void pack_kernel(const float* __restrict__ src, T* __restrict__ dst, int mode, int taps, int cin, int cout, int kpad, int npad) {
  const int ptaps = (mode >= 2) ? 1 : taps;
  const long long total = (long long)ptaps * (kpad / EL) * npad;
  for (long long it = blockIdx.x * (long long)blockDim.x + threadIdx.x; it < total; it += (long long)gridDim.x * blockDim.x) {
    const int nn = (int)(it % npad);
    const int k8 = (int)((it / npad) % (kpad / EL));
    const int tap = (int)(it / ((long long)npad * (kpad / EL)));
    float v[EL];
#pragma unroll
    for (int e = 0; e < EL; ++e) {
      const int k = k8 * EL + e;
      float x = 0.f;
      if (mode == 0) { if (k < cin && nn < cout) x = src[((size_t)tap * cin + k) * cout + nn]; }
      else if (mode == 1) { if (k < cout && nn < cin) x = src[((size_t)(taps - 1 - tap) * cin + nn) * cout + k]; }
      else if (mode == 2) { if (k < cin && nn < taps * cout) x = src[(size_t)nn * cin + k]; }
      else { if (k < taps * cout && nn < cin) x = src[(size_t)k * cin + nn]; }
      v[e] = x;
    }
    if constexpr (EL == 8) {
      store8<T>(dst + it * 8, v);
    } else {
      float lo[8], hi[8];
#pragma unroll
      for (int e = 0; e < 8; ++e) { lo[e] = v[e]; hi[e] = v[8 + e]; }
      store8<T>(dst + it * 16, lo);
      store8<T>(dst + it * 16 + 8, hi);
    }
  }
}
template <typename T>
__global__ __launch_bounds__(EW_BLOCK) void pack_batched_kernel(const satcv_pack_job* __restrict__ jobs, const long long* __restrict__ prefix, int njobs, long long total) {
  for (long long g0 = (long long)blockIdx.x * EW_BLOCK; g0 < total; g0 += (long long)gridDim.x * EW_BLOCK) {
    int lo = 0, hi = njobs - 1;
    while (lo < hi) { const int mid = (lo + hi + 1) >> 1; if (prefix[mid] <= g0) lo = mid; else hi = mid - 1; }
    lo = __builtin_amdgcn_readfirstlane(lo);
    const satcv_pack_job j = jobs[lo];
    long long it = g0 - prefix[lo] + threadIdx.x;
    const long long real = (long long)(j.mode >= 2 ? 1 : j.taps) * (j.kpad / 8) * j.npad;
    if (it >= real) continue;
    if (j.mode == 1 && (j.kpad / 8) % 4 == 0 && j.npad % 16 == 0) {
      const int nb = j.npad / 16, kb = (j.kpad / 8) / 4;
      const int l = (int)(it % 64); long long t = it / 64;
      const int nblk = (int)(t % nb); t /= nb;
      const int kblk = (int)(t % kb); const long long tap_ = t / kb;
      const int k8_ = kblk * 4 + (l & 3), nn_ = nblk * 16 + (l >> 2);
      it = (tap_ * (j.kpad / 8) + k8_) * j.npad + nn_;
    }
    const int nn = (int)(it % j.npad);
    const int k8 = (int)((it / j.npad) % (j.kpad / 8));
    const int tap = (int)(it / ((long long)j.npad * (j.kpad / 8)));
    float v[8];
#pragma unroll
    for (int e = 0; e < 8; ++e) {
      const int k = k8 * 8 + e;
      float x = 0.f;
      if (j.mode == 0) { if (k < j.cin && nn < j.cout) x = j.src[((size_t)tap * j.cin + k) * j.cout + nn]; }
      else if (j.mode == 1) { if (k < j.cout && nn < j.cin) x = j.src[((size_t)(j.taps - 1 - tap) * j.cin + nn) * j.cout + k]; }
      else if (j.mode == 2) { if (k < j.cin && nn < j.taps * j.cout) x = j.src[(size_t)nn * j.cin + k]; }
      else { if (k < j.taps * j.cout && nn < j.cin) x = j.src[(size_t)k * j.cin + nn]; }
      v[e] = x;
    }
    store8<T>(reinterpret_cast<T*>(j.dst) + it * 8, v);
  }
}
extern "C" int64_t satcv_pack_job_items(const satcv_pack_job* j) {
  if (!j || j->kpad <= 0 || j->kpad % 8 || j->npad <= 0 || j->mode < 0 || j->mode > 3) return -1;
  const int64_t real = (int64_t)(j->mode >= 2 ? 1 : j->taps) * (j->kpad / 8) * j->npad;
  return (real + EW_BLOCK - 1) / EW_BLOCK * EW_BLOCK;
}
extern "C" int satcv_pack_weights_batched(const satcv_pack_job* jobs_dev, const int64_t* prefix_dev, int32_t njobs, int64_t total_items, int32_t dtype,
                                          void* stream) {
  SATCV_CHECK(jobs_dev && prefix_dev && njobs > 0 && total_items > 0, "pack_weights_batched: bad args");
  SATCV_CHECK(total_items % EW_BLOCK == 0, "pack_weights_batched: the prefix table must be built from satcv_pack_job_items (multiples of 256)");
  DISPATCH_T8(dtype, hipLaunchKernelGGL(pack_batched_kernel<T>, dim3(ew_grid(total_items)), dim3(EW_BLOCK), 0, (hipStream_t)stream, jobs_dev,
                                        (const long long*)prefix_dev, njobs, (long long)total_items));
  LAUNCH_OK("pack_weights_batched");
  return SATCV_OK;
}

extern "C" int satcv_pack_weights(const float* src, void* dst_fwd, void* dst_dgrad, int32_t kh, int32_t kw, int32_t cin, int32_t cout, int32_t cin_pad, int32_t transposed, int32_t dtype, void* stream) {
  SATCV_CHECK(src && cin > 0 && cout > 0 && cin_pad >= cin && cin_pad % 16 == 0, "pack_weights: bad args");
  const int taps = kh * kw;
  hipStream_t st = (hipStream_t)stream;
  if (dtype == SATCV_FP8X) {
    SATCV_CHECK(dst_fwd && !dst_dgrad && cin_pad % 16 == 0, "pack_weights: the scaled fp8 image is forward-only, cin_pad %% 16 == 0");
    const int kp = cin_pad, np = rup(transposed ? taps * cout : cout, 32);
    const long long items = (long long)(transposed ? 1 : taps) * (kp / 16) * np;
    hipLaunchKernelGGL((pack_kernel<fp8, 16>), dim3(ew_grid(items)), dim3(EW_BLOCK), 0, st, src, (fp8*)dst_fwd, transposed ? 2 : 0, taps, cin, cout, kp, np);
    LAUNCH_OK("pack_weights");
    return SATCV_OK;
  }
  DISPATCH_T8(dtype, {
    if (!transposed) {
      if (dst_fwd) { const int kp = cin_pad, np = rup(cout, 32);
        hipLaunchKernelGGL(pack_kernel<T>, dim3(ew_grid((long long)taps * (kp / 8) * np)), dim3(EW_BLOCK), 0, st, src, (T*)dst_fwd, 0, taps, cin, cout, kp, np); }
      if (dst_dgrad) { const int kp = rup(cout, 16), np = rup(cin, 32);
        hipLaunchKernelGGL(pack_kernel<T>, dim3(ew_grid((long long)taps * (kp / 8) * np)), dim3(EW_BLOCK), 0, st, src, (T*)dst_dgrad, 1, taps, cin, cout, kp, np); }
    } else {
      if (dst_fwd) { const int kp = cin_pad, np = rup(taps * cout, 32);
        hipLaunchKernelGGL(pack_kernel<T>, dim3(ew_grid((long long)(kp / 8) * np)), dim3(EW_BLOCK), 0, st, src, (T*)dst_fwd, 2, taps, cin, cout, kp, np); }
      if (dst_dgrad) { const int kp = rup(taps * cout, 16), np = rup(cin, 32);
        hipLaunchKernelGGL(pack_kernel<T>, dim3(ew_grid((long long)(kp / 8) * np)), dim3(EW_BLOCK), 0, st, src, (T*)dst_dgrad, 3, taps, cin, cout, kp, np); }
    }
  });
  LAUNCH_OK("pack_weights");
  return SATCV_OK;
}

__global__ void bn_finalize_train_kernel(satcv_stat_t* stats, int ld, int c, float count, const float* gamma, const float* beta,
                                         float eps, float momentum, int updates, int bessel, float* mm, float* mv,
// ... 1440 lines not shown
  const long long n4 = n / 4;
  for (long long i = blockIdx.x * (long long)blockDim.x + threadIdx.x; i < n4; i += (long long)gridDim.x * blockDim.x) {
    float4 pp = reinterpret_cast<float4*>(p)[i];
    const float4 gg = reinterpret_cast<const float4*>(g)[i];
    float4 mm = reinterpret_cast<float4*>(m)[i];
    float4 vv = reinterpret_cast<float4*>(v)[i];
    float4 lm = lr_mul ? reinterpret_cast<const float4*>(lr_mul)[i] : make_float4(1.f, 1.f, 1.f, 1.f);
    float* P = &pp.x; const float* Gp = &gg.x; float* M = &mm.x; float* V = &vv.x; const float* L = &lm.x;
#pragma unroll
    for (int e = 0; e < 4; ++e) {
      const float gr = Gp[e] * gs;
      const float mn = b1 * M[e] + (1.f - b1) * gr;
      const float vn = b2 * V[e] + (1.f - b2) * gr * gr;
      if (L[e] != 0.f) { M[e] = mn; V[e] = vn; P[e] -= L[e] * alpha * mn / (sqrtf(vn) + eps); }
    }
    reinterpret_cast<float4*>(p)[i] = pp; reinterpret_cast<float4*>(m)[i] = mm; reinterpret_cast<float4*>(v)[i] = vv;
  }
  if (blockIdx.x == 0 && threadIdx.x < (n & 3)) {
    const long long i = n4 * 4 + threadIdx.x;
    const float l = lr_mul ? lr_mul[i] : 1.f;
    const float gr = g[i] * gs;
    const float mn = b1 * m[i] + (1.f - b1) * gr, vn = b2 * v[i] + (1.f - b2) * gr * gr;
    if (l != 0.f) { m[i] = mn; v[i] = vn; p[i] -= l * alpha * mn / (sqrtf(vn) + eps); }
  }
}
__global__ void adam_bump_kernel(float* state) { state[1] += 1.f; }
__global__ __launch_bounds__(256) void zero2_kernel(uint4* __restrict__ a, long long na16, unsigned* __restrict__ b, long long nb4) {
  const uint4 z = make_uint4(0u, 0u, 0u, 0u);
  for (long long i = blockIdx.x * (long long)blockDim.x + threadIdx.x; i < na16; i += (long long)gridDim.x * blockDim.x) a[i] = z;
  if (blockIdx.x == 0) for (long long i = threadIdx.x; i < nb4; i += blockDim.x) b[i] = 0u;
}
extern "C" int satcv_zero2(void* a, int64_t bytes_a, void* b, int64_t bytes_b, void* stream) {
  SATCV_CHECK(bytes_a >= 0 && bytes_b >= 0 && (bytes_a == 0 || a) && (bytes_b == 0 || b), "zero2: bad args");
  SATCV_CHECK(((uintptr_t)a % 16 == 0) && bytes_a % 16 == 0 && ((uintptr_t)b % 4 == 0) && bytes_b % 4 == 0, "zero2: a must be 16-byte, b 4-byte aligned and sized");
  if (bytes_a == 0 && bytes_b == 0) return SATCV_OK;
  hipLaunchKernelGGL(zero2_kernel, dim3(ew_grid(bytes_a / 16 + 1, 4096)), dim3(256), 0, (hipStream_t)stream, reinterpret_cast<uint4*>(a), (long long)(bytes_a / 16),
                     reinterpret_cast<unsigned*>(b), (long long)(bytes_b / 4));
  LAUNCH_OK("zero2");
  return SATCV_OK;
}
extern "C" int satcv_adam_step_part(float* p, const float* g, float* m, float* v, int64_t n, float beta1, float beta2, float eps, float* state,
                                    const float* lr_mul, int32_t bump, void* stream) {
  SATCV_CHECK(p && g && m && v && state && n > 0, "adam: bad args");
  SATCV_CHECK(((uintptr_t)p % 16 == 0) && ((uintptr_t)g % 16 == 0) && ((uintptr_t)m % 16 == 0) && ((uintptr_t)v % 16 == 0), "adam: buffers must be 16-byte aligned");
  hipLaunchKernelGGL(adam_kernel, dim3(ew_grid(n / 4 + 1, 4096)), dim3(EW_BLOCK), 0, (hipStream_t)stream, p, g, m, v, (long long)n, beta1, beta2, eps, state, lr_mul);
  if (bump) hipLaunchKernelGGL(adam_bump_kernel, dim3(1), dim3(1), 0, (hipStream_t)stream, state);
  LAUNCH_OK("adam");
  return SATCV_OK;
}
extern "C" int satcv_adam_step(float* p, const float* g, float* m, float* v, int64_t n, float beta1, float beta2, float eps, float* state,
                               const float* lr_mul, void* stream) {
  SATCV_CHECK(p && g && m && v && state && n > 0, "adam: bad args");
  SATCV_CHECK(((uintptr_t)p % 16 == 0) && ((uintptr_t)g % 16 == 0) && ((uintptr_t)m % 16 == 0) && ((uintptr_t)v % 16 == 0), "adam: buffers must be 16-byte aligned");
  hipLaunchKernelGGL(adam_kernel, dim3(ew_grid(n / 4 + 1, 4096)), dim3(EW_BLOCK), 0, (hipStream_t)stream, p, g, m, v, (long long)n, beta1, beta2, eps, state, lr_mul);
  hipLaunchKernelGGL(adam_bump_kernel, dim3(1), dim3(1), 0, (hipStream_t)stream, state);
  LAUNCH_OK("adam");
  return SATCV_OK;
}
```

### satellite_computervision_amd/csrc/igemm_common.hpp

```cpp
#pragma once
#include "common.hpp"

struct IgemmArgs {
  const void* x0; const void* x1;
  int c0, c1;
  const float* in_scale; const float* in_shift; int in_relu;
  const void* w; const float* bias; const float* out_scale;
  void* pool_y; int pool_ld, pool_f;
  void* y; int ldy;
  satcv_stat_t* stats; int stats_ld;
  int n, h, w_;
  int hs, ws;
  int cout, cout_pad;
  int kh, kw, dil;
  int mode_in, mode_out, f;
  int cstat, out_relu, accumulate, stride;
  int tiles_x, tiles_y, ngroups;
  int rpi, imgs, seg, rl, cl, pitch, halh, halw;
  int n_tiles;
  int nchunks;
  int halh_tl, halw_tl;
  int taploop, cpt;
  const void* bst_y; const void* bst_y1; int bst_ld, bst_ld1, bst_split;
  const float* bst_scale; const float* bst_shift; const float* bst_mean; const float* bst_rstd; int bst_relu;
  int dbg;
  int ksplit; float* kslab;
  int tile_policy;
  int pair_n, pair_c0, pair_c1;
};

template <typename T>
struct FragT;
template <>
struct FragT<bf16> { bf16x8 v; };
template <>
struct FragT<float> { float4 lo, hi; };
template <>
struct FragT<fp8> { long v; };
template <>
struct FragT<fp8s> { i32x4 lo, hi; };

template <typename T>
__device__ __forceinline__ FragT<T> lds_frag(const T* p, int sub_stride = 0) {
  FragT<T> f;
  if constexpr (std::is_same<T, fp8s>::value) {
    f.lo = *reinterpret_cast<const i32x4*>(p);
    f.hi = *reinterpret_cast<const i32x4*>(p + sub_stride);
  } else if constexpr (std::is_same<T, bf16>::value) {
    f.v = *reinterpret_cast<const bf16x8*>(p);
  } else if constexpr (std::is_same<T, fp8>::value) {
    f.v = *reinterpret_cast<const long*>(p);
  } else {
    f.lo = reinterpret_cast<const float4*>(p)[0];
    f.hi = reinterpret_cast<const float4*>(p)[1];
  }
  return f;
}

template <typename T>
__device__ __forceinline__ void mma32(f32x16& acc, const FragT<T>& a, const FragT<T>& b) {
  if constexpr (std::is_same<T, bf16>::value) {
// ... 433 lines not shown
```

### satellite_computervision_amd/engine.py

```python
import ctypes as C
import os
import itertools
from collections import defaultdict
from fractions import Fraction

import numpy as np
import torch

from . import ops, parallel
from ._lib import lib, check, F32, BF16, STAT_ROWS

_M16_DEFAULT = int(os.environ.get('SATCV_M16', '1'))

BN_EPS = 1e-3
BN_MOMENTUM = 0.99


class KTensor:
    _ids = itertools.count()

    def __init__(self, node, channels, down=Fraction(1), name=None):
        self.id = next(KTensor._ids)
        self.node, self.channels, self.down, self.name = node, channels, down, name

# ... 30 lines not shown
EARLY_OPT = os.environ.get('SATCV_EARLY_OPT', '0') == '1'
EARLY_OPT_FRAC = 0.05
FUSE_DGRAD_ALL = os.environ.get('SATCV_FUSE_DGRAD_BN_BWD', '1') == '2'


def rup(a, b):
    return (a + b - 1) // b * b


def topo_nodes(outputs):
    seen, order = set(), []

    def visit(node):
        if id(node) in seen:
            return
        seen.add(id(node))
        for t in node.inputs:
            visit(t.node)
        order.append(node)
    for t in outputs:
        visit(t.node)
    return order


class TRef:

    def __init__(self, srcs, n, h, w, affine=None, relu=False):
        self.srcs, self.n, self.h, self.w = srcs, n, h, w
        self.affine, self.relu = affine, relu

    @property
    def c(self):
        return sum(c for _, c in self.srcs)


def _fp(t, off=0):
    return None if t is None else t.data_ptr() + t.element_size() * off


class Runtime:

    def __init__(self, model, dtype):
        if not torch.cuda.is_available():
            raise RuntimeError('satellite_computervision_amd needs a ROCm GPU (no CPU fallback)')
        self.model, self.dtype = model, dtype
        self.tdtype = ops.TORCH_DTYPE[dtype]
        self.esize = 2 if dtype == BF16 else 4
        self.dev = torch.device('cuda', torch.cuda.current_device())
        self.offsets = {}
        off = 0
        for p in model.param_specs:
            if p.kind in ('moving_mean', 'moving_var'):
                continue
            self.offsets[p.name] = off
            off += rup(p.size, 4)
        self.n_train = off
        soff = 0
        self.soffsets = {}
        for p in model.param_specs:
            if p.kind in ('moving_mean', 'moving_var'):
                self.soffsets[p.name] = soff
                soff += rup(p.size, 4)
        self.pflat = torch.zeros(max(off, 4), dtype=torch.float32, device=self.dev)
        self.gflat = torch.zeros_like(self.pflat)
        self.sflat = torch.zeros(max(soff, 4), dtype=torch.float32, device=self.dev)
        self.adam_m = self.adam_v = None
# ... 59 lines not shown
    def _note_gamma(self, name, v):
        if name.endswith('/gamma'):
            bn = name[:-len('/gamma')]
            if np.any(np.abs(v) < np.finfo(np.float32).tiny):
                self.zero_gamma.add(bn)
            else:
                self.zero_gamma.discard(bn)

    def _pack_table(self, lo=0, hi=None):
        from ._lib import PackJob
        jobs = []
        for lname, pk in self.packed.items():
            if not (lo <= self.offsets[lname + '/kernel'] < (self.n_train if hi is None else hi)):
                continue
            taps, cin, cout, cp = pk['k'][0] * pk['k'][1], pk['cin'], pk['cout'], pk['cin_pad']
            src = self.pptr(lname + '/kernel')
            if not pk['transposed']:
                jobs.append(PackJob(src, pk['fwd'].data_ptr(), 0, taps, cin, cout, cp, rup(cout, 32)))
                jobs.append(PackJob(src, pk['dgrad'].data_ptr(), 1, taps, cin, cout, rup(cout, 16), rup(cin, 32)))
            else:
                jobs.append(PackJob(src, pk['fwd'].data_ptr(), 2, taps, cin, cout, cp, rup(taps * cout, 32)))
                jobs.append(PackJob(src, pk['dgrad'].data_ptr(), 3, taps, cin, cout, rup(taps * cout, 16), rup(cin, 32)))
        if not jobs:
            return None
        prefix, tot = [], 0
        for j in jobs:
            prefix.append(tot)
            tot += int(lib.satcv_pack_job_items(C.byref(j)))
        arr = (PackJob * len(jobs))(*jobs)
        raw = torch.frombuffer(bytearray(bytes(arr)), dtype=torch.uint8).to(self.dev)
        pre = torch.tensor(prefix, dtype=torch.int64, device=self.dev)
        return dict(jobs=raw, prefix=pre, n=len(jobs), total=tot)

    def repack(self, lo=0, hi=None, stream=None):
        if not self.packed:
            return
        key = (lo, hi)
        if key not in self._ptabs:
            self._ptabs[key] = self._pack_table(lo, hi)
        t = self._ptabs[key]
        if t is None:
            return
        check(lib.satcv_pack_weights_batched(t['jobs'].data_ptr(), t['prefix'].data_ptr(), t['n'], t['total'], self.dtype,
                                             ops.stream_ptr() if stream is None else stream))

    def ensure_adam(self):
        if self.adam_m is None:
            self.adam_m = torch.zeros_like(self.pflat)
            self.adam_v = torch.zeros_like(self.pflat)

    def plan(self, n, h, w, training):
        frozen = tuple(sorted(l.name for l in self.model.layers if not l.trainable)) if training else ()
        raw_bn = tuple(sorted(self.zero_gamma)) if training else ()
        key = (n, h, w, bool(training), frozen, raw_bn)
        if key not in self.plans:
            self.plans[key] = Plan(self, n, h, w, training, frozen, raw_bn)
        return self.plans[key]


class Plan:

    def __init__(self, rt, n, h, w, training, frozen=(), raw_bn=()):
        self.rt, self.n, self.h, self.w, self.training = rt, n, h, w, training
        self.frozen = set(frozen)
        self.raw_bn = set(raw_bn)
        self.tile_policy = 2 if (training and _M16_DEFAULT == 1) else 0
        self.eo_lo, self.early_opt, self.eo_done = None, None, False
        self.fwd, self.bwd = [], []
        self.keep = []
        self.dropouts = []
        self.x_inputs = []
        self.x_by_tid = {}
        self.x_src = {}
        _sp = os.environ.get('SATCV_SIDE_PRIORITY')
        self.side = (torch.cuda.Stream(priority=int(_sp)) if _sp is not None else torch.cuda.Stream()) if (training and rt.model.wgrad_side_stream) else None
        self.step_count = 0
        self.outputs = {}
        self.sync_bn = bool(training and getattr(rt.model, 'sync_bn', False) and parallel.active())
        self.amax_of = {}
        self._bn_jobs = []
        self._build()
        if self._bn_jobs:
            tab = torch.tensor([[int(v or 0) for v in j] for j in self._bn_jobs], dtype=torch.int64).to(rt.dev)
            self.keep.append(tab)
            nj = len(self._bn_jobs)
            self.fwd.insert(0, lambda st: check(lib.satcv_bn_affine_infer_batched(tab.data_ptr(), nj, BN_EPS, st)))

    def _z(self, *shape, dtype=None):
        t = torch.zeros(*shape, dtype=dtype or self.rt.tdtype, device=self.rt.dev)
        self.keep.append(t)
        return t

    def _dims(self, t):
        hh, ww = self.h * t.down, self.w * t.down
        if hh.denominator != 1 or ww.denominator != 1:
            raise ValueError(f'input {self.h}x{self.w} is not divisible by the model downsampling ({1 / t.down})')
        return int(hh), int(ww)

    def _conv_step(self, role='fwd', **kw):
        kw.setdefault('tile_policy', self.tile_policy)
        d = ops.make_conv_desc(**kw)
        self.keep.append(d)
        fn = lambda st, d=d: check(lib.satcv_conv2d_igemm(C.byref(d), st))
        k, cin, cout = kw.get('kh', 1) * kw.get('kw', 1), kw.get('c0', 0) + (kw.get('c1', 0) or 0), kw['cout']
        px = kw['n'] * kw['h'] * kw['w_']
        fn.label = (f"conv_{role} k{kw.get('kh', 1)} d{kw.get('dil', 1)} n{kw['n']} {kw['h']}x{kw['w_']} {kw.get('c0', 0)}+{kw.get('c1', 0) or 0}->{cout}"
                    f"{' d2s' if kw.get('mode_out') else ''}{' s2d' if kw.get('mode_in') else ''}")
        fn.work = dict(kind='conv', role=role, taps=k, px=px, cin=cin, cout=cout, esize=self.rt.esize)
        return fn

    def _src_args(self, r):
        (x0, c0) = r.srcs[0]
        x1, c1 = (r.srcs[1] if len(r.srcs) > 1 else (None, 0))
        a = r.affine
        return dict(x0=x0.data_ptr(), c0=c0, x1=x1.data_ptr() if x1 is not None else None, c1=c1,
                    in_scale=_fp(a['scale']) if a else None, in_shift=_fp(a['shift']) if a else None,
                    in_relu=1 if (a and r.relu) else 0)

    def _bn_forward(self, bnname, stats, ld, off, c, count, updates, aff=None, aoff=0, conv_bias=None, bias_eff=None):
        rt = self.rt
        a = aff or dict(scale=self._z(c, dtype=torch.float32), shift=self._z(c, dtype=torch.float32),
                        mean=self._z(c, dtype=torch.float32), rstd=self._z(c, dtype=torch.float32))
        g, b = rt.pptr(bnname + '/gamma'), rt.pptr(bnname + '/beta')
        mm, mv = rt.sptr(bnname + '/moving_mean'), rt.sptr(bnname + '/moving_var')
        if self.training:
            bessel = 1 if rt.model.bn_bessel else 0
            if self.sync_bn:
                self.fwd.append(lambda st: parallel.allreduce_mean_(stats))
            if bnname in self.frozen:
                ts, tt = self._z(c, dtype=torch.float32), self._z(c, dtype=torch.float32)
                self.fwd.append(lambda st: check(lib.satcv_bn_finalize_train(
                    _fp(stats, off), ld, c, float(count), g, b, BN_EPS, BN_MOMENTUM, updates, bessel, None, None,
                    _fp(ts), _fp(tt), _fp(a['mean'], aoff), _fp(a['rstd'], aoff), st)))
                self.fwd.append(lambda st: check(lib.satcv_bn_affine_infer(g, b, mm, mv, BN_EPS, c, _fp(a['scale'], aoff), _fp(a['shift'], aoff), st)))
                return a
            self.fwd.append(lambda st: check(lib.satcv_bn_finalize_train(
# ... 2 lines not shown
        else:
            self._bn_jobs.append((g, b, mm, mv, _fp(a['scale'], aoff), _fp(a['shift'], aoff), c, conv_bias, bias_eff))
        return a

    def _materialize(self, t, r, f=1, pooled=None, sink=None, actslot=None):
        if not r.relu:
            raise NotImplementedError('materialising a linear (no-ReLU) BatchNorm output')
        (y, c) = r.srcs[0]
        hh, ww = r.h, r.w
        if actslot is None:
            act = self._z(self.n, hh, ww, c)
            act_ptr, act_ld = act.data_ptr(), c
        else:
            act = actslot[0]
            act_ptr, act_ld = actslot[0].data_ptr() + actslot[1] * self.rt.esize, actslot[2]
        st_ptr, ld = (None, 0)
        if sink is not None and self.training:
            st_ptr, ld = _fp(sink[0], sink[1]), sink[2]
        a = r.affine
        dt = self.rt.dtype
        if (self.training and pooled is not None and f == 2 and dt == BF16 and getattr(self.rt.model, 'fuse_pool_bwd', True)
                and hh % 8 == 0 and ww % 32 == 0 and c in (32, 64)):
            amax = self._z(self.n, hh // 2, ww // 2, c, dtype=torch.uint8)
            self.amax_of[t.id] = amax
            self.fwd.append(lambda st: check(lib.satcv_bn_relu_pool_amax(
                y.data_ptr(), _fp(a['scale']), _fp(a['shift']), act_ptr, act_ld, pooled.data_ptr(), amax.data_ptr(),
                st_ptr, ld, self.n, hh, ww, c, f, dt, st)))
            return TRef([(act, c)], self.n, hh, ww) if actslot is None else None
        self.fwd.append(lambda st: check(lib.satcv_bn_relu_pool(
            y.data_ptr(), _fp(a['scale']), _fp(a['shift']), act_ptr, act_ld, pooled.data_ptr() if pooled is not None else None,
            st_ptr, ld, self.n, hh, ww, c, f, dt, st)))
        return TRef([(act, c)], self.n, hh, ww) if actslot is None else None

    def _build(self):
        rt, m, n = self.rt, self.rt.model, self.n
        T, dt, es = rt.tdtype, rt.dtype, rt.esize
        training = self.training
        consumers = defaultdict(list)
        for node in m.nodes:
            for t in node.inputs:
                consumers[t.id].append(node)
        vals, acts, ctx = {}, {}, {}
        sinks, cat_stats = {}, {}
        order = {id(nd): i for i, nd in enumerate(m.nodes)}
        fused_join = {}
        folded_plain = {}
        for node in m.nodes:
            if node.op == 'concat_bn_relu':
                a, b = node.inputs
                ctot = a.channels + b.channels
                st = self._z(STAT_ROWS, 2, ctot, dtype=torch.float64)
                cat_stats[id(node)] = st
                sinks[a.id] = (st, 0, ctot)
                sinks[b.id] = (st, a.channels, ctot)

        slots, actslots = {}, {}
        for node in m.nodes:
            if node.op == 'concat':
                if all(t.node.op == 'cba' and len(consumers[t.id]) > 1 for t in node.inputs):
                    ctot = sum(t.channels for t in node.inputs)
                    hh, ww = self._dims(node.inputs[0])
                    shared = self._z(n, hh, ww, ctot)
                    off = 0
                    for t in node.inputs:
                        actslots[t.id] = (shared, off, ctot)
                        if node.outputs[0].id in sinks:
                            st_, so_, sl_ = sinks[node.outputs[0].id]
                            sinks[t.id] = (st_, so_ + off, sl_)
                        off += t.channels
                    ctx[id(node)] = dict(act=shared, ctot=ctot)
                    continue
                if not all(t.node.op == 'cba' and len(consumers[t.id]) == 1 for t in node.inputs):
                    raise NotImplementedError('concatenate is supported for conv_batch_act outputs consumed only by the concat (ASPP)')
                ctot = sum(t.channels for t in node.inputs)
                hh, ww = self._dims(node.inputs[0])
                yshared = self._z(n, hh, ww, ctot)
                stshared = self._z(STAT_ROWS, 2, ctot, dtype=torch.float64) if training else None
                aff = dict(scale=self._z(ctot, dtype=torch.float32), shift=self._z(ctot, dtype=torch.float32),
                           mean=self._z(ctot, dtype=torch.float32), rstd=self._z(ctot, dtype=torch.float32))
                off = 0
                for t in node.inputs:
                    slots[t.id] = dict(y=yshared, off=off, ctot=ctot, stats=stshared, aff=aff)
                    off += t.channels
                ctx[id(node)] = dict(y=yshared, ctot=ctot, aff=aff)

        for node in m.nodes:
            op = node.op
            if op == 'input':
                t = node.outputs[0]
                cp = rup(t.channels, 16)
                x = self._z(n, self.h, self.w, cp)
                xin = self._z(n, self.h, self.w, t.channels, dtype=torch.float32)
                self.x_f32 = xin
                self.x_inputs.append(xin)
                self.x_by_tid[t.id] = xin
                npix = n * self.h * self.w
                cc = t.channels
                self.fwd.append(lambda st, xin=xin, x=x, npix=npix, cc=cc, cp=cp, tid=t.id: check(lib.satcv_ingest_nhwc(
                    self.x_src.get(tid) or xin.data_ptr(), x.data_ptr(), npix, cc, cp, dt, st)))
                vals[t.id] = TRef([(x, cp)], n, self.h, self.w)
            elif op == 'cba':
                tin, tout = node.inputs[0], node.outputs[0]
                r = vals[tin.id]
                lay = node.layer
                pk = rt.packed[lay.name]
                cout = tout.channels
                if cout % 16:
                    raise NotImplementedError(f'{lay.name}: filters must be a multiple of 16 (got {cout})')
                if r.c != pk['cin_pad']:
                    raise ValueError(f'{lay.name}: input has {r.c} stored channels, kernel expects {pk["cin_pad"]}')
                k, dil = node.attrs['k'], node.attrs['dil']
                stride, relu_out = node.attrs.get('stride', 1), node.attrs.get('relu', True)
                hin, win = r.h, r.w
                if stride > 1:
                    if training:
                        raise NotImplementedError('strided convolutions are inference-only (DeepLab backbone)')
                    r = TRef(r.srcs, r.n, (hin - 1) // stride + 1, (win - 1) // stride + 1, r.affine, r.relu)
                sl = slots.get(tout.id)
                if not node.attrs.get('bn', True):
                    if sl is not None or stride > 1:
                        raise NotImplementedError('a convolution without BatchNormalization as a concatenation branch / with a stride')
                    y = self._z(n, r.h, r.w, cout)
                    self.fwd.append(self._conv_step(w=pk['fwd'].data_ptr(), bias=rt.pptr(lay.name + '/bias'), y=y.data_ptr(), ldy=cout, n=n, h=r.h, w_=r.w,
                                                    cout=cout, cout_pad=rup(cout, 32), kh=k, kw=k, dil=dil, dtype=dt, **self._src_args(r)))
                    vals[tout.id] = TRef([(y, cout)], n, r.h, r.w)
                    ctx[id(node)] = dict(r=r, y=y, yoff=0, ldy=cout, aff=None, aoff=0, cout=cout, k=k, dil=dil)
                    continue
                join = consumers[tout.id][0] if (not training and sl is None and not relu_out and FUSE_RESIDUAL
                                                 and len(consumers[tout.id]) == 1 and consumers[tout.id][0].op == 'add_relu'
                                                 and tout in consumers[tout.id][0].inputs) else None
                if join is not None:
                    tsc = join.inputs[1] if join.inputs[0] is tout else join.inputs[0]
# ... 5 lines not shown
                            y = self._z(n, r.h, r.w, cout)
                            fold_args = dict(y=y.data_ptr(), accumulate=0)
                            folded_plain[tout.id] = y
                            sb = y
                    else:
                        src_ok = (tsc.id in folded_plain) or (tsc.node is not None and tsc.node.op == 'add_relu' and stride == 1)
                        if (src_ok and not rs_.affine and len(rs_.srcs) == 1 and rs_.srcs[0][1] == cout and rs_.srcs[0][0].shape[-1] == cout
                                and (rs_.h, rs_.w) == (r.h, r.w)
                                and all(cn is join or order[id(cn)] < order[id(node)] for cn in consumers[tsc.id])):
                            sb = rs_.srcs[0][0]
                            fold_args = dict(y=sb.data_ptr(), accumulate=2)
                            fused_join[id(join)] = sb
                    if fold_args is not None:
                        be = self._z(cout, dtype=torch.float32)
                        aff = self._bn_forward(lay.bn_name, None, cout, 0, cout, n * r.h * r.w, node.attrs.get('bn_updates', 1),
                                               conv_bias=rt.pptr(lay.name + '/bias'), bias_eff=_fp(be))
                        self.fwd.append(self._conv_step(w=pk['fwd'].data_ptr(), bias=_fp(be), out_scale=_fp(aff['scale']), ldy=cout,
                                                        n=n, h=r.h, w_=r.w, cout=cout, cout_pad=rup(cout, 32), kh=k, kw=k, dil=dil, dtype=dt,
                                                        stride=stride, hin=hin if stride > 1 else 0, win=win if stride > 1 else 0,
                                                        **fold_args, **self._src_args(r)))
                        vals[tout.id] = TRef([(sb, cout)], n, r.h, r.w)
                        ctx[id(node)] = dict(r=r, y=sb, yoff=0, ldy=cout, aff=None, aoff=0, cout=cout, k=k, dil=dil)
                        continue
                if sl is None:
                    y = self._z(n, r.h, r.w, cout)
                    stats = self._z(STAT_ROWS, 2, cout, dtype=torch.float64) if training else None
                    yoff, ldy, aoff, aff_in = 0, cout, 0, None
                else:
                    y, stats, yoff, ldy, aoff, aff_in = sl['y'], sl['stats'], sl['off'], sl['ctot'], sl['off'], sl['aff']
                self.fwd.append(self._conv_step(w=pk['fwd'].data_ptr(), bias=rt.pptr(lay.name + '/bias'), y=y.data_ptr() + yoff * es, ldy=ldy,
                                                stats=_fp(stats, aoff), stats_ld=ldy, n=n, h=r.h, w_=r.w, cout=cout, cout_pad=rup(cout, 32),
                                                kh=k, kw=k, dil=dil, dtype=dt, stride=stride, hin=hin if stride > 1 else 0,
                                                win=win if stride > 1 else 0, **self._src_args(r)))
                aff = self._bn_forward(lay.bn_name, stats, ldy, aoff, cout, n * r.h * r.w, node.attrs.get('bn_updates', 1), aff_in, aoff)
                if sl is None:
                    vals[tout.id] = TRef([(y, cout)], n, r.h, r.w, affine=aff, relu=relu_out)
                ctx[id(node)] = dict(r=r, y=y, yoff=yoff, ldy=ldy, aff=aff, aoff=aoff, cout=cout, k=k, dil=dil)
            elif op == 'concat':
                cx = ctx[id(node)]
                hh, ww = self._dims(node.inputs[0])
                if 'act' in cx:
                    vals[node.outputs[0].id] = TRef([(cx['act'], cx['ctot'])], n, hh, ww)
                else:
                    vals[node.outputs[0].id] = TRef([(cx['y'], cx['ctot'])], n, hh, ww, affine=cx['aff'], relu=True)
            elif op == 'pool':
                tin, tout = node.inputs[0], node.outputs[0]
                r = vals[tin.id]
                f = node.attrs['f']
                if not (r.affine and len(r.srcs) == 1):
                    raise NotImplementedError('max-pool expects the output of a conv_batch_act block')
                c = r.c
                if r.h % f or r.w % f:
                    raise ValueError(f'input {self.h}x{self.w} is not divisible by the model downsampling (a {r.h}x{r.w} map meets a {f}x{f} pool)')
                pooled = self._z(n, r.h // f, r.w // f, c)
                others = [cn for cn in consumers[tin.id] if cn is not node]
                if others:
                    acts[tin.id] = self._materialize(tin, r, f, pooled, sinks.get(tin.id), actslots.get(tin.id))
                else:
                    (y, _) = r.srcs[0]
                    a = r.affine
                    hh, ww = r.h, r.w
                    self.fwd.append(lambda st, y=y, a=a, pooled=pooled, hh=hh, ww=ww, c=c, f=f: check(lib.satcv_bn_relu_pool(
                        y.data_ptr(), _fp(a['scale']), _fp(a['shift']), None, 0, pooled.data_ptr(), None, 0, n, hh, ww, c, f, dt, st)))
                vals[tout.id] = TRef([(pooled, c)], n, r.h // f, r.w // f)
                ctx[id(node)] = dict(f=f)
            elif op == 'convT':
# ... 626 lines not shown
                if (amax is not None and getattr(rt.model, 'fuse_pool_bwd', True) and dt == ops.BF16 and da is not None and dp is not None
                        and gpool_f.get(tout.id, 1) == 2 and not graws and not BIAS_NOISE and cx['k'] == 3 and cx['dil'] == 1 and da[2] == ldy
                        and dp[1] == 0 and lay.bn_name not in self.frozen and gact.get(tin.id) is None and lay.name not in shared_layers):
                    pkp = rt.packed[lay.name]
                    sa = self._src_args(r)
                    want_dx = tin.node.op != 'input'
                    cinp = r.c
                    ginp = self._z(n, hh, ww, cinp) if want_dx else None
                    fzp = ops.make_bwdf_desc(g=da_ptr, yraw=y.data_ptr() + yoff * es, ldg=ldy, bn_scale=_fp(aff['scale'], aoff), bn_shift=_fp(aff['shift'], aoff),
                                             bn_mean=_fp(aff['mean'], aoff), bn_rstd=_fp(aff['rstd'], aoff), bn_coef=_fp(app.coef), linear=0,
                                             w_dgrad=pkp['dgrad'].data_ptr() if want_dx else None, dx=ginp.data_ptr() if want_dx else None,
                                             lddx=cinp if want_dx else 0, dw=rt.gptr(lay.name + '/kernel'), cin=pkp['cin'], cout=cout, n=n, h=hh, w_=ww,
                                             dtype=dt, accumulate=accum, dpool=dp[0].data_ptr(), lddp=dp[2], amax=amax.data_ptr(), **sa)
                    ent = None
                    if (want_dx and POOL_SUMS and tin.node.op == 'pool' and len(consumers[tin.id]) == 1 and sa['in_scale'] is None
                            and len(vals[tin.id].srcs) == 1 and tin.node.inputs[0].channels == cinp):
                        ent = act_sums_for(tin.node.inputs[0])
                    if ent is not None:
                        fzp.bst_sums, fzp.bst_sums_ld, fzp.bst_act_form = _fp(ent['buf']), cinp, 1
                    nbp = lib.satcv_conv2d_bwd_fused_workspace(C.byref(fzp))
                    if nbp < 0:
                        fzp = None
                    elif ent is not None:
                        ent['parts'].add('pool')
                if fzp is not None:
                    if DEFER and not accum and lay.name not in shared_layers:
                        fzp.defer_reduce = 1
                        fzp._own_ws = nbp
                        rpending.append((fzp, 'f', 4 * 9 * pkp['cin'] * cout))
                    else:
                        fused_ws_need = max(fused_ws_need, nbp)
                    fdescs.append(fzp)
                    self.keep.append(fzp)
                    self.bwd += [fin] if (pre is not None or red is None) else [red, fin]
                    fstep = lambda st, fzp=fzp: check(lib.satcv_conv2d_bwd_fused(C.byref(fzp), st))
                    fstep.label = f"bwd_fused k3 n{n} {hh}x{ww} {sa['c0']}+{sa['c1']}->{cout} pooled{'' if want_dx else ' nodx'}{' +poolsums' if fzp.bst_sums else ''}"
                    fstep.work = dict(kind='bwd_fused', taps=9, px=n * hh * ww, cin=pkp['cin'], cout=cout, esize=es, nodx=not want_dx, pooled=True)
                    self.bwd.append(fstep)
                    if want_dx:
                        gact[tin.id] = (ginp, 0, cinp)
                        self.dbg['dx:' + lay.name] = ginp
                    self.dbg['dyparts:' + lay.name] = dict(g=da, y=y, yoff=yoff, ldy=ldy, aff=aff, aoff=aoff, cout=cout, coef=app.coef, linear=0,
                                                           dp=dp, amax=amax)
                    self.dbg['_ctx:' + lay.name] = dict(da=da, dp=dp, y=y, yoff=yoff, ldy=ldy, aff=aff, aoff=aoff, cout=cout)
                    continue
                self.bwd += [fin, app] if (pre is not None or red is None) else [red, fin, app]
                for gr in graws:
                    if gr[1] != 0 or gr[2] != cout:
                        raise NotImplementedError('raw-output gradient in a channel slice')
                    bpart = self._z(max(lib.satcv_bias_grad_workspace(n * hh * ww, cout) // 4, 1), dtype=torch.float32)
                    self.bwd.append(lambda st, dy=dy, gb=gr[0], npx=n * hh * ww, cout=cout, db=rt.gptr(lay.name + '/bias'), bpart=bpart: (
                        check(lib.satcv_bias_grad(gb.data_ptr(), cout, npx, cout, dt, db, bpart.data_ptr(), st)),
                        check(lib.satcv_add_act(dy.data_ptr(), None, None, gb.data_ptr(), None, None, 0, dy.data_ptr(), npx, cout, dt, st))))
                self.dbg['dy:' + lay.name] = dy
                self.dbg['_ctx:' + lay.name] = dict(da=da, dp=dp, y=y, yoff=yoff, ldy=ldy, aff=aff, aoff=aoff, cout=cout)
                pk = rt.packed[lay.name]
                wstep = wgrad_step(r, dy.data_ptr(), cout, lay, pk['cin'], cout, hh, ww, cx['k'], cx['dil'], accum=accum,
                                   last=tin.node.op == 'input' and len(m.inputs) == 1 and os.environ.get('SATCV_WGRAD_LAST_FULL', '1') != '0')
                if not WGRAD_LATE:
                    self.bwd.append(wstep)
                if tin.node.op != 'input':
                    cinp = r.c
                    prev = gact.get(tin.id)
                    if prev is not None and (prev[1] != 0 or prev[2] != cinp):
                        raise NotImplementedError('gradient fan-in into a channel slice')
                    gin = prev[0] if prev is not None else self._z(n, hh, ww, cinp)
# ... 201 lines not shown
```

### satellite_computervision_amd/model_tools.py

```python
import ctypes as C
import json
import os
import time
from collections import defaultdict
from fractions import Fraction

import numpy as np
import torch

from . import engine as E
from . import ops
from ._lib import lib, check, F32, BF16

_DEFAULT_DTYPE = 'bfloat16'
_RNG = np.random.default_rng(0)
_UIDS = defaultdict(int)


def set_compute_dtype(name):
    global _DEFAULT_DTYPE
    assert name in ('bfloat16', 'float32')
    _DEFAULT_DTYPE = name


# ... 1081 lines not shown
        if isinstance(yb, torch.Tensor):
            if _resident_f32(yb, plan.y_true):
                plan.y_src = yb
            else:
                plan.y_true.copy_(yb.to(torch.float32), non_blocking=True)
        else:
            plan.y_true.copy_(torch.from_numpy(np.ascontiguousarray(yb, dtype=np.float32)), non_blocking=True)

    def train_step_device(self, xb, yb, sync_grads=None):
        if self._loss is None:
            raise RuntimeError('compile() the model before fit/train')
        rt = self.runtime
        rt.ensure_adam()
        n, h, w, _ = self._shape_of(xb)
        plan = self._head_plan(n, h, w, True)
        if getattr(self, '_frozen_applied', None) != plan.frozen:
            self._apply_trainable()
            self._frozen_applied = plan.frozen
        self._stage_x(plan, xb)
        self._stage_y(plan, yb)
        st = ops.stream_ptr()
        check(lib.satcv_zero2(rt.gflat.data_ptr(), rt.gflat.numel() * 4 // 16 * 16, plan.loss_buf.data_ptr(), 4, st))
        if rt.gflat.numel() % 4:
            rt.gflat[rt.gflat.numel() // 4 * 4:].zero_()
        plan.step_count += 1
        plan.run_forward(st)
        self._loss_launch(plan, st)
        opt = self.optimizer
        plan.eo_done = False
        plan.early_opt = dict(beta_1=opt.beta_1, beta_2=opt.beta_2, epsilon=opt.epsilon) if sync_grads is None else None
        plan.run_backward(st)
        if sync_grads is not None:
            sync_grads(rt.gflat)
        if plan.eo_done:
            lo = plan.eo_lo
            check(lib.satcv_adam_step_part(rt.pflat.data_ptr(), rt.gflat.data_ptr(), rt.adam_m.data_ptr(), rt.adam_v.data_ptr(), lo,
                                           opt.beta_1, opt.beta_2, opt.epsilon, rt.adam_state.data_ptr(),
                                           rt.lr_mul.data_ptr() if rt.lr_mul is not None else None, 1, st))
            rt.repack(0, lo)
        else:
            check(lib.satcv_adam_step(rt.pflat.data_ptr(), rt.gflat.data_ptr(), rt.adam_m.data_ptr(), rt.adam_v.data_ptr(), rt.pflat.numel(),
                                      opt.beta_1, opt.beta_2, opt.epsilon, rt.adam_state.data_ptr(),
                                      rt.lr_mul.data_ptr() if rt.lr_mul is not None else None, st))
            rt.repack()
        self._weights_version = getattr(self, '_weights_version', 0) + 1
        return plan

    def train_on_batch(self, x, y):
        plan = self.train_step_device(x, y, getattr(self, '_sync_grads', None))
        return float(plan.loss_buf.item())

    def _metric_values(self, conf, loss):
        vals = [loss]
        conf = conf.astype(np.float64)
        for mt in self._metrics:
            if isinstance(mt, str):
                vals.append(float(np.trace(conf) / max(conf.sum(), 1)))
            else:
                tp = np.diag(conf)
                denom = conf.sum(0) + conf.sum(1) - tp
                valid = denom > 0
                vals.append(float((tp[valid] / denom[valid]).mean()) if valid.any() else 0.0)
        return vals

    def _run_epoch(self, batches, steps, train):
        rt = self.runtime
        loss_sum = torch.zeros(1, dtype=torch.float32, device=rt.dev)
        conf, cnt = None, 0
        sync = getattr(self, '_sync_grads', None)
        if steps is not None:
            import itertools as _it
            batches = _it.islice(batches, steps)
        for i, b in enumerate(_prefetch_to_device(batches, rt.dev)):
            if steps is not None and i >= steps:
                break
            xb, yb = b[0], b[1]
            if train:
# ... 252 lines not shown
```

### satellite_computervision_amd/ops.py

```python
import ctypes as C
import torch

from . import _lib
from ._lib import lib, check, ConvDesc, WgradDesc, BnBwdDesc, HeadDesc, F32, BF16, FP8, FP8X, STAT_ROWS

TORCH_DTYPE = {F32: torch.float32, BF16: torch.bfloat16, FP8: torch.float8_e4m3fn, FP8X: torch.float8_e4m3fn}
DTYPE_CODE = {torch.float32: F32, torch.bfloat16: BF16, torch.float8_e4m3fn: FP8}


def rup(a, b):
    return (a + b - 1) // b * b


def stream_ptr():
    return C.c_void_p(torch.cuda.current_stream().cuda_stream)


def ptr(t):
    if t is None:
        return None
    assert t.is_cuda, 'satcv ops need device tensors (no CPU fallback)'
    return C.c_void_p(t.data_ptr())


# ... 59 lines not shown
    d.out_relu, d.dtype, d.accumulate = int(out_relu), dtype, int(accumulate)
    d.stride, d.hin, d.win, d.out_scale = stride, hin, win, out_scale
    d.pool_y, d.pool_ld, d.pool_f = pool_y, pool_ld, pool_f
    if bst:
        d.bst_y, d.bst_ld, d.bst_y1, d.bst_ld1, d.bst_split = bst['y'], bst['ld'], bst.get('y1'), bst.get('ld1', 0), bst.get('split', 0)
        d.bst_scale, d.bst_shift, d.bst_mean, d.bst_rstd, d.bst_relu = bst['scale'], bst['shift'], bst['mean'], bst['rstd'], int(bst.get('relu', 1))
    return d


def _p(t):
    return t.data_ptr() if t is not None else None


def conv2d(x, w_packed, cout, *, kh=3, kw=3, dil=1, bias=None, x1=None, in_scale=None, in_shift=None, in_relu=False,
           stats=None, out=None, out_relu=False, stride=1, bst=None, out_scale=None, pool_y=None, pool_f=0):
    n, hin, win, c0 = x.shape
    h, w_ = ((hin - 1) // stride + 1, (win - 1) // stride + 1) if stride > 1 else (hin, win)
    dtype = DTYPE_CODE[x.dtype]
    c1 = x1.shape[-1] if x1 is not None else 0
    cpad = rup(cout, 32)
    y = out if out is not None else torch.empty(n, h, w_, rup(cout, 16), dtype=x.dtype, device=x.device)
    d = make_conv_desc(x0=_p(x), c0=c0, x1=_p(x1), c1=c1, w=_p(w_packed), y=_p(y), ldy=y.shape[-1], n=n, h=h, w_=w_,
                       cout=cout, cout_pad=cpad, dtype=dtype, in_scale=_p(in_scale), in_shift=_p(in_shift),
                       in_relu=in_relu, bias=_p(bias), stats=_p(stats), stats_ld=stats.shape[-1] if stats is not None else 0,
                       kh=kh, kw=kw, dil=dil, out_relu=out_relu, stride=stride, hin=hin if stride > 1 else 0, win=win if stride > 1 else 0,
                       out_scale=_p(out_scale), pool_y=_p(pool_y), pool_ld=pool_y.shape[-1] if pool_y is not None else 0, pool_f=pool_f,
                       bst={k: (_p(v) if torch.is_tensor(v) else v) for k, v in bst.items()} if bst else None)
    if bst and lib.satcv_conv2d_igemm_pipelined(C.byref(d)) != 1:
        raise ValueError('conv2d: this shape cannot carry the fused BatchNorm-backward reduce (bst); run satcv_bn_bwd_reduce separately')
    check(lib.satcv_conv2d_igemm(C.byref(d), stream_ptr()))
    return y


def conv2d_transpose(x, w_packed, cout, f, *, bias=None, in_scale=None, in_shift=None, in_relu=False, stats=None, out=None,
                     out_scale=None, out_relu=False):
    n, h, w_, c0 = x.shape
    dtype = DTYPE_CODE[x.dtype]
    y = out if out is not None else torch.empty(n, h * f, w_ * f, rup(cout, 16), dtype=x.dtype, device=x.device)
    d = make_conv_desc(x0=_p(x), c0=c0, w=_p(w_packed), y=_p(y), ldy=y.shape[-1], n=n, h=h, w_=w_, cout=f * f * cout,
                       cout_pad=rup(f * f * cout, 32), dtype=dtype, in_scale=_p(in_scale), in_shift=_p(in_shift),
                       in_relu=in_relu, bias=_p(bias), stats=_p(stats), stats_ld=stats.shape[-1] if stats is not None else 0,
                       kh=1, kw=1, dil=1, mode_out=1, f=f, cstat=cout, out_scale=_p(out_scale), out_relu=out_relu)
    check(lib.satcv_conv2d_igemm(C.byref(d), stream_ptr()))
    return y


def conv2d_dgrad(dy, w_dgrad, cin, *, kh=3, kw=3, dil=1, out=None, accumulate=False):
    n, h, w_, cy = dy.shape
    dtype = DTYPE_CODE[dy.dtype]
    dx = out if out is not None else torch.empty(n, h, w_, rup(cin, 16), dtype=dy.dtype, device=dy.device)
    d = make_conv_desc(x0=_p(dy), c0=cy, w=_p(w_dgrad), y=_p(dx), ldy=dx.shape[-1], n=n, h=h, w_=w_, cout=cin,
                       cout_pad=rup(cin, 32), dtype=dtype, kh=kh, kw=kw, dil=dil, accumulate=accumulate)
    check(lib.satcv_conv2d_igemm(C.byref(d), stream_ptr()))
    return dx


def conv2d_transpose_dgrad(dy, w_dgrad, cin, cout, f, *, out=None, stats=None, bst=None):
    n, hf, wf, cy = dy.shape
    h, w_ = hf // f, wf // f
    dtype = DTYPE_CODE[dy.dtype]
    assert cy == cout, 'dy channel stride must equal cout'
    dx = out if out is not None else torch.empty(n, h, w_, rup(cin, 16), dtype=dy.dtype, device=dy.device)
    d = make_conv_desc(x0=_p(dy), c0=cy, w=_p(w_dgrad), y=_p(dx), ldy=dx.shape[-1], n=n, h=h, w_=w_, cout=cin,
                       cout_pad=rup(cin, 32), dtype=dtype, kh=1, kw=1, dil=1, mode_in=1, f=f,
                       stats=_p(stats), stats_ld=stats.shape[-1] if stats is not None else 0,
                       bst={k: (_p(v) if torch.is_tensor(v) else v) for k, v in bst.items()} if bst else None)
    check(lib.satcv_conv2d_igemm(C.byref(d), stream_ptr()))
    return dx


def make_wgrad_desc(*, x0, c0, dy, lddy, dw, cin, cout, n, h, w_, dtype, x1=None, c1=0, in_scale=None, in_shift=None,
                    in_relu=0, kh=3, kw=3, dil=1, mode_dy=0, f=1, transposed=0, workspace=None, workspace_bytes=0, accumulate=0, whole_chip=0, defer_reduce=0):
    d = WgradDesc()
    d.x0, d.x1, d.c0, d.c1 = x0, x1, c0, c1
    d.in_scale, d.in_shift, d.in_relu = in_scale, in_shift, int(in_relu)
    d.dy, d.lddy, d.dw, d.cin, d.cout = dy, lddy, dw, cin, cout
    d.n, d.h, d.w_, d.kh, d.kw, d.dil = n, h, w_, kh, kw, dil
    d.mode_dy, d.f, d.transposed = mode_dy, f, transposed
    d.workspace, d.workspace_bytes, d.dtype, d.accumulate = workspace, workspace_bytes, dtype, int(accumulate)
    d.whole_chip = int(whole_chip)
    d.defer_reduce = int(defer_reduce)
    return d


def make_bwdf_desc(*, g, yraw, ldg, bn_scale, bn_shift, bn_mean, bn_rstd, bn_coef, x0, c0, w_dgrad, dx, lddx, dw, cin, cout, n, h, w_, dtype,
                   linear=0, x1=None, c1=0, in_scale=None, in_shift=None, in_relu=0, kh=3, kw=3, dil=1, workspace=None, workspace_bytes=0,
                   accumulate=0, bst_sums=None, bst_sums_ld=0, bst_mean=None, bst_rstd=None, bst_act_form=0, dpool=None, lddp=0, amax=None,
                   hg_dlogits=None, hg_w=None, hg_ncls=0):
    from ._lib import BwdfDesc
    d = BwdfDesc()
    d.g, d.yraw, d.ldg = g, yraw, ldg
    d.bn_scale, d.bn_shift, d.bn_mean, d.bn_rstd, d.bn_coef, d.linear = bn_scale, bn_shift, bn_mean, bn_rstd, bn_coef, int(linear)
    d.x0, d.x1, d.c0, d.c1 = x0, x1, c0, c1
    d.in_scale, d.in_shift, d.in_relu = in_scale, in_shift, int(in_relu)
    d.w_dgrad, d.dx, d.lddx, d.dw, d.cin, d.cout = w_dgrad, dx, lddx, dw, cin, cout
    d.n, d.h, d.w_, d.kh, d.kw, d.dil = n, h, w_, kh, kw, dil
    d.workspace, d.workspace_bytes, d.dtype, d.accumulate = workspace, workspace_bytes, dtype, int(accumulate)
    d.bst_sums, d.bst_sums_ld, d.bst_mean, d.bst_rstd, d.bst_act_form = bst_sums, bst_sums_ld, bst_mean, bst_rstd, int(bst_act_form)
    d.dpool, d.lddp, d.amax = dpool, lddp, amax
    d.hg_dlogits, d.hg_w, d.hg_ncls = hg_dlogits, hg_w, int(hg_ncls)
    return d


def conv_bwd_fused(g, yraw, scale, shift, mean, rstd, coef, x, w_dgrad, cin, cout, *, x1=None, in_scale=None, in_shift=None, in_relu=False,
                   linear=False, accumulate_into=None, bst=None, dpool=None, amax=None, want_dx=True, head=None):
    n, h, w_, c0 = x.shape
    c1 = x1.shape[-1] if x1 is not None else 0
    dx = torch.empty(n, h, w_, c0 + c1, dtype=x.dtype, device=x.device) if want_dx else None
    dw = accumulate_into if accumulate_into is not None else torch.empty(3, 3, cin, cout, dtype=torch.float32, device=x.device)
    d = make_bwdf_desc(g=_p(g), yraw=_p(yraw), ldg=g.shape[-1] if g is not None else yraw.shape[-1], bn_scale=_p(scale), bn_shift=_p(shift), bn_mean=_p(mean), bn_rstd=_p(rstd),
                       bn_coef=_p(coef), x0=_p(x), c0=c0, x1=_p(x1), c1=c1, in_scale=_p(in_scale), in_shift=_p(in_shift), in_relu=in_relu,
                       w_dgrad=_p(w_dgrad), dx=_p(dx), lddx=c0 + c1, dw=_p(dw), cin=cin, cout=cout, n=n, h=h, w_=w_, dtype=DTYPE_CODE[x.dtype],
                       linear=linear, accumulate=accumulate_into is not None, dpool=_p(dpool), lddp=dpool.shape[-1] if dpool is not None else 0,
                       amax=_p(amax), **(dict(hg_dlogits=_p(head[0]), hg_w=_p(head[1]), hg_ncls=head[0].shape[-1]) if head else {}),
                       **(dict(bst_sums=_p(bst['sums']), bst_sums_ld=bst['sums'].shape[-1], bst_mean=_p(bst.get('mean')), bst_rstd=_p(bst.get('rstd')),
                               bst_act_form=bst.get('act_form', 0)) if bst else {}))
    nb = lib.satcv_conv2d_bwd_fused_workspace(C.byref(d))
    if nb < 0:
        return None
    ws = torch.empty(max(nb // 4, 1), dtype=torch.float32, device=x.device)
    d.workspace, d.workspace_bytes = ws.data_ptr(), nb
    check(lib.satcv_conv2d_bwd_fused(C.byref(d), stream_ptr()))
    return dx, dw


def conv2d_wgrad(x, dy, cin, cout, *, kh=3, kw=3, dil=1, x1=None, in_scale=None, in_shift=None, in_relu=False,
                 transposed_f=0, dw=None):
    n, h, w_, c0 = x.shape
    dtype = DTYPE_CODE[x.dtype]
    c1 = x1.shape[-1] if x1 is not None else 0
    f = transposed_f
    if dw is None:
        shape = (f, f, cout, cin) if f else (kh, kw, cin, cout)
        dw = torch.empty(shape, dtype=torch.float32, device=x.device)
    d = make_wgrad_desc(x0=_p(x), c0=c0, x1=_p(x1), c1=c1, dy=_p(dy), lddy=dy.shape[-1], dw=_p(dw), cin=cin, cout=cout,
                        n=n, h=h, w_=w_, dtype=dtype, in_scale=_p(in_scale), in_shift=_p(in_shift), in_relu=in_relu,
                        kh=1 if f else kh, kw=1 if f else kw, dil=dil, mode_dy=1 if f else 0, f=f if f else 1,
                        transposed=1 if f else 0)
    nbytes = lib.satcv_conv2d_wgrad_workspace(C.byref(d))
    if nbytes < 0:
        raise _lib.SatcvError(lib.satcv_last_error().decode())
    ws = torch.empty(max(nbytes // 4, 1), dtype=torch.float32, device=x.device)
    d.workspace, d.workspace_bytes = ws.data_ptr(), nbytes
    check(lib.satcv_conv2d_wgrad(C.byref(d), stream_ptr()))
    return dw


def bn_finalize_train(stats, count, gamma, beta, moving_mean, moving_var, eps=1e-3, momentum=0.99, updates=1, bessel=False):
    c = gamma.numel()
    dev = gamma.device
    scale, shift, mean, rstd = (torch.empty(c, dtype=torch.float32, device=dev) for _ in range(4))
    check(lib.satcv_bn_finalize_train(ptr(stats), stats.shape[-1], c, float(count), ptr(gamma), ptr(beta), eps, momentum,
                                      updates, int(bessel), ptr(moving_mean), ptr(moving_var), ptr(scale), ptr(shift),
# ... 200 lines not shown
```

Measured before the change: 8235 tiles/s.

## Read fp32 model input directly in first conv and fold Adam bump into repack

Adds a direct-input mode in which the first 3x3 conv's forward (weights-stationary igemm) and its fused backward read the 4-channel fp32 input tile straight from the source, converting it to bf16 and zero-padding to 16 channels in registers. This removes the separate ingest pass and the padded bf16 copy of the input. It also merges the Adam step-counter bump into the batched weight-repack launch, which drops a small kernel per step. The cost is more template variants and special-case guards, and the feature only applies when the input shape and alignment match.

```diff
diff --git a/include/satcv.h b/include/satcv.h
--- a/include/satcv.h
+++ b/include/satcv.h
@@ -31,6 +31,8 @@
 int64_t satcv_pack_job_items(const satcv_pack_job* job);
 int satcv_pack_weights_batched(const satcv_pack_job* jobs_dev, const int64_t* prefix_dev, int32_t njobs, int64_t total_items, int32_t dtype,
                                void* stream);
+int satcv_pack_weights_batched_bump(const satcv_pack_job* jobs_dev, const int64_t* prefix_dev, int32_t njobs, int64_t total_items, int32_t dtype,
+                                    float* adam_state, void* stream);
 
 typedef struct satcv_conv_desc {
   const void* x0;
@@ -116,6 +118,7 @@
   const void* dpool; int32_t lddp; const void* amax;
   const float* hg_dlogits; const float* hg_w; int32_t hg_ncls;
   int32_t defer_reduce;
+  const float* x0_f32; int32_t x0_c;
 } satcv_bwdf_desc;
 int64_t satcv_conv2d_bwd_fused_workspace(const satcv_bwdf_desc* d);
 int satcv_conv2d_bwd_fused(const satcv_bwdf_desc* d, void* stream);
diff --git a/satellite_computervision_amd/_lib.py b/satellite_computervision_amd/_lib.py
--- a/satellite_computervision_amd/_lib.py
+++ b/satellite_computervision_amd/_lib.py
@@ -81,7 +81,7 @@
                 ('workspace', c_vp), ('workspace_bytes', c_i64), ('dtype', c_i32), ('accumulate', c_i32),
                 ('bst_sums', c_vp), ('bst_sums_ld', c_i32), ('bst_mean', c_vp), ('bst_rstd', c_vp), ('bst_act_form', c_i32),
                 ('dpool', c_vp), ('lddp', c_i32), ('amax', c_vp),
-                ('hg_dlogits', c_vp), ('hg_w', c_vp), ('hg_ncls', c_i32), ('defer_reduce', c_i32)]
+                ('hg_dlogits', c_vp), ('hg_w', c_vp), ('hg_ncls', c_i32), ('defer_reduce', c_i32), ('x0_f32', c_vp), ('x0_c', c_i32)]
 
 
 class CtbfDesc(C.Structure):
@@ -155,6 +155,7 @@
     'satcv_pack_weights': (C.c_int, [c_vp, c_vp, c_vp, c_i32, c_i32, c_i32, c_i32, c_i32, c_i32, c_i32, c_vp]),
     'satcv_pack_job_items': (c_i64, [C.POINTER(PackJob)]),
     'satcv_pack_weights_batched': (C.c_int, [c_vp, c_vp, c_i32, c_i64, c_i32, c_vp]),
+    'satcv_pack_weights_batched_bump': (C.c_int, [c_vp, c_vp, c_i32, c_i64, c_i32, c_vp, c_vp]),
     'satcv_conv2d_igemm': (C.c_int, [C.POINTER(ConvDesc), c_vp]),
     'satcv_conv2d_igemm_pipelined': (C.c_int, [C.POINTER(ConvDesc)]),
     'satcv_conv2d_wgrad_workspace': (c_i64, [C.POINTER(WgradDesc)]),
diff --git a/satellite_computervision_amd/csrc/api.hip b/satellite_computervision_amd/csrc/api.hip
--- a/satellite_computervision_amd/csrc/api.hip
+++ b/satellite_computervision_amd/csrc/api.hip
@@ -130,6 +130,7 @@
 int g_opt_m16p_prio = env_int("SATCV_M16P_PRIO", 30);
 int g_opt_wgrad_m16 = env_int("SATCV_WGRAD_M16", 0);
 int g_opt_splitk = env_int("SATCV_SPLITK", 0);
+int g_opt_direct_input = 1;
 static int* opt_slot(const char* key) {
   if (!key) return nullptr;
   if (!strcmp(key, "igemm_db")) return &g_opt_igemm_db;
@@ -144,6 +145,7 @@
   if (!strcmp(key, "m16p_prio")) return &g_opt_m16p_prio;
   if (!strcmp(key, "wgrad_m16")) return &g_opt_wgrad_m16;
   if (!strcmp(key, "m16p_launches")) return &g_m16p_launches;
+  if (!strcmp(key, "direct_input")) return &g_opt_direct_input;
   return nullptr;
 }
 extern "C" int satcv_set_option(const char* key, int32_t value) {
diff --git a/satellite_computervision_amd/csrc/common.hpp b/satellite_computervision_amd/csrc/common.hpp
--- a/satellite_computervision_amd/csrc/common.hpp
+++ b/satellite_computervision_amd/csrc/common.hpp
@@ -252,6 +252,17 @@
   return o;
 }
 
+__device__ __forceinline__ Raw8<bf16> f32x4_to_bf16_item(const Raw8<bf16>& raw) {
+  const float4 f = __builtin_bit_cast(float4, raw.q[0]);
+  bf16x8 w;
+  w[0] = (bf16)f.x; w[1] = (bf16)f.y; w[2] = (bf16)f.z; w[3] = (bf16)f.w;
+#pragma unroll
+  for (int e = 4; e < 8; ++e) w[e] = (bf16)0.f;
+  Raw8<bf16> o;
+  o.q[0] = __builtin_bit_cast(uint4, w);
+  return o;
+}
+
 template <typename T>
 __device__ __forceinline__ float round_to(float x) {
   if constexpr (std::is_same<T, bf16>::value) return (float)(bf16)x;
diff --git a/satellite_computervision_amd/csrc/conv_bwd_fused.hip b/satellite_computervision_amd/csrc/conv_bwd_fused.hip
--- a/satellite_computervision_amd/csrc/conv_bwd_fused.hip
+++ b/satellite_computervision_amd/csrc/conv_bwd_fused.hip
@@ -25,6 +25,7 @@
   int bst_act_form;
   const void* dp; int lddp; const unsigned char* amax;
   const float* hg_dl; const float* hg_w;
+  const float* x0_f32;
 };
 
 __device__ __forceinline__ bf16x4 tr_read4(const bf16* p) {
@@ -32,9 +33,10 @@
   return __builtin_bit_cast(bf16x4, v);
 }
 
-template <int CIN, int COUT, int NW, int WPS, bool POOL = false, bool NODG = false, int CINS = CIN, bool HG = false>
+template <int CIN, int COUT, int NW, int WPS, bool POOL = false, bool NODG = false, int CINS = CIN, bool HG = false, bool XF32 = false>
 __global__ __launch_bounds__(NW * 64, WPS) void bwd_fused_kernel(const BwdfArgs a, const int total_tiles) {
   static_assert(!HG || !POOL, "the head feeds a decoder block");
+  static_assert(!XF32 || (NODG && CINS == 16), "the fp32 source is the 4-channel model input: no data gradient, 16 presented channels");
   typedef bf16 T;
   constexpr int TW = 32, TH = 8, BM = 256, RL = TH + 2, CL = TW + 2, PITCH = CL, EL = 8, NTHREADS = NW * 64;
   constexpr int SD = COUT / 8, SX = CIN / 8, SXR = CINS / 8;
@@ -113,9 +115,10 @@
   const int g_rowstride = a.e.w_ * a.ldg;
   const unsigned gy_lane = (unsigned)slot_d * EL;
   const int xch0 = slot_x * EL;
-  const bool xsecond = xch0 >= a.c0;
-  const T* xsrc = xsecond ? reinterpret_cast<const T*>(a.x1) + (xch0 - a.c0) : reinterpret_cast<const T*>(a.x0) + xch0;
-  const int xcs = xsecond ? a.c1 : a.c0;
+  const bool xsecond = !XF32 && xch0 >= a.c0;
+  const T* xsrc = XF32 ? reinterpret_cast<const T*>(a.x0_f32)
+                       : (xsecond ? reinterpret_cast<const T*>(a.x1) + (xch0 - a.c0) : reinterpret_cast<const T*>(a.x0) + xch0);
+  const int xcs = XF32 ? 8 : (xsecond ? a.c1 : a.c0);
   const int xq0 = tid / SXR;
   const int x_l0 = slot_x * XSTRIDE + xq0 * EL;
   const int x_eoff0 = ((xq0 / TW) * a.e.w_ + (xq0 % TW)) * xcs, x_estep = (XPIX_STEP / TW) * a.e.w_ * xcs;
@@ -292,6 +295,7 @@
 #pragma unroll
       for (int j = 0; j < XI; ++j) {
         Raw8<T> v = rx[j];
+        if constexpr (XF32) v = select8<T>(slot_x == 0, f32x4_to_bf16_item(v));
         if (xaff) v = affine8_lim(v, sc, sh, xrelu_lim);
         lstore8<T>(ldsX + x_l0 + j * (XPIX_STEP * EL), v);
       }
@@ -506,8 +510,10 @@
   return (int)grid;
 }
 
+extern int g_opt_direct_input;
 static bool bwdf_shape_ok(const satcv_bwdf_desc* d, int& cin_s) {
   cin_s = d->c0 + d->c1;
+  if (d->x0_f32 && (!g_opt_direct_input || d->x0_c != 4 || d->c0 != 16 || d->x1 || d->in_scale || d->dx || !d->dpool || ((uintptr_t)d->x0_f32 % 16) != 0)) return false;
   if (d->dtype != SATCV_BF16 || d->kh != 3 || d->kw != 3 || d->dil != 1) return false;
   if (d->x1 && d->c0 % 8 != 0) return false;
   if (d->h % 8 != 0 || d->w_ % 32 != 0) return false;
@@ -527,7 +533,7 @@
   return true;
 }
 
-template <int CIN, int COUT, int NW, int WPS, bool POOL = false, bool NODG = false, int CINS = CIN, bool HG = false>
+template <int CIN, int COUT, int NW, int WPS, bool POOL = false, bool NODG = false, int CINS = CIN, bool HG = false, bool XF32 = false>
 static int bwdf_launch(const satcv_bwdf_desc* d, hipStream_t st, bool query, int64_t* ws_bytes, satcv_reduce_job* job = nullptr) {
   using G = BwdfGeom<CIN, COUT, NW, NODG>;
   static_assert(G::LDS <= 160 * 1024, "tile + weights exceed the LDS");
@@ -549,7 +555,8 @@
   a.bst_sums = d->bst_sums; a.bst_ld = d->bst_sums_ld; a.bst_mean = d->bst_mean; a.bst_rstd = d->bst_rstd; a.bst_act_form = d->bst_act_form;
   a.dp = d->dpool; a.lddp = d->lddp; a.amax = reinterpret_cast<const unsigned char*>(d->amax);
   a.hg_dl = d->hg_dlogits; a.hg_w = d->hg_w;
-  auto kern = bwd_fused_kernel<CIN, COUT, NW, WPS, POOL, NODG, CINS, HG>;
+  a.x0_f32 = d->x0_f32;
+  auto kern = bwd_fused_kernel<CIN, COUT, NW, WPS, POOL, NODG, CINS, HG, XF32>;
   { const int rc = satcv_ensure_dynamic_lds(reinterpret_cast<const void*>(kern), G::LDS); if (rc) return rc; }
   const double flops = (NODG ? 2.0 : 4.0) * d->n * d->h * d->w_ * (double)CINS * COUT * 9;
   satcv_prof_begin(3, flops, st);
@@ -566,8 +573,10 @@
   if (!bwdf_shape_ok(d, cin_s)) return SATCV_ERR_UNSUPPORTED;
   if (d->dpool) {
     if (d->dx) return bwdf_launch<32, 64, 4, 1, true, false>(d, st, query, ws_bytes, job);
+    if (d->x0_f32) return bwdf_launch<32, 32, 8, 2, true, true, 16, false, true>(d, st, query, ws_bytes, job);
     return bwdf_launch<32, 32, 8, 2, true, true, 16>(d, st, query, ws_bytes, job);
   }
+  if (d->x0_f32) return SATCV_ERR_UNSUPPORTED;
   if (cin_s == 32 && d->hg_dlogits) return bwdf_launch<32, 32, 8, 2, false, false, 32, true>(d, st, query, ws_bytes, job);
   if (d->hg_dlogits) return SATCV_ERR_UNSUPPORTED;
   if (cin_s == 32) return bwdf_launch<32, 32, 8, 2>(d, st, query, ws_bytes, job);
@@ -587,7 +596,7 @@
 }
 
 extern "C" int satcv_conv2d_bwd_fused(const satcv_bwdf_desc* d, void* stream) {
-  SATCV_CHECK(d && (d->g || d->hg_dlogits) && d->yraw && d->x0 && d->dw && d->workspace && (d->dx == nullptr || d->w_dgrad), "bwd_fused: null pointer");
+  SATCV_CHECK(d && (d->g || d->hg_dlogits) && d->yraw && (d->x0 || d->x0_f32) && d->dw && d->workspace && (d->dx == nullptr || d->w_dgrad), "bwd_fused: null pointer");
   SATCV_CHECK(d->bn_scale && d->bn_shift && d->bn_mean && d->bn_rstd && d->bn_coef, "bwd_fused: BatchNorm coefficients missing");
   SATCV_CHECK((d->c1 == 0) == (d->x1 == nullptr) && d->n > 0 && d->h > 0 && d->w_ > 0, "bwd_fused: bad dims");
   SATCV_CHECK(!d->bst_sums || (d->bst_sums_ld >= d->c0 + d->c1 && (d->bst_act_form ? d->in_scale == nullptr
diff --git a/satellite_computervision_amd/csrc/conv_igemm.hip b/satellite_computervision_amd/csrc/conv_igemm.hip
--- a/satellite_computervision_amd/csrc/conv_igemm.hip
+++ b/satellite_computervision_amd/csrc/conv_igemm.hip
@@ -264,6 +264,8 @@
 
 static int igemm_fill_args(const satcv_conv_desc* d, IgemmArgs& a) {
   SATCV_CHECK(d && d->x0 && d->w && d->y, "igemm: null pointer");
+  const bool direct = d->mode_in == 2;
+  const int mode_in = direct ? 0 : d->mode_in;
   SATCV_CHECK(d->c0 > 0 && d->c0 % 16 == 0 && d->c1 % 16 == 0, "igemm: channels must be multiples of 16 (c0=%d c1=%d)", d->c0, d->c1);
   SATCV_CHECK(d->dtype != SATCV_FP8X || (d->c0 % 64 == 0 && d->c1 % 64 == 0 && !d->in_scale), "igemm: the scaled fp8 path needs channels %% 64 == 0 and no input transform");
   SATCV_CHECK((d->c1 == 0) == (d->x1 == nullptr), "igemm: x1/c1 mismatch");
@@ -273,9 +275,9 @@
               d->kh <= 15 && d->kw <= 15 && d->dil <= (1 << 15) && d->f <= 16 && d->stride <= 16,
               "igemm: extents out of range (n*h*w must stay below 2^31 pixels, channels below 2^20)");
   SATCV_CHECK(d->cstat > 0, "igemm: cstat");
-  SATCV_CHECK((!d->mode_in && !d->mode_out) || (d->f >= 2 && d->kh == 1 && d->kw == 1), "igemm: s2d/d2s need 1x1 taps and f>=2");
+  SATCV_CHECK((!mode_in && !d->mode_out) || (d->f >= 2 && d->kh == 1 && d->kw == 1), "igemm: s2d/d2s need 1x1 taps and f>=2");
   SATCV_CHECK(!(d->accumulate && d->stats), "igemm: accumulate with statistics");
-  SATCV_CHECK(!(d->mode_in && d->in_scale), "igemm: s2d source cannot carry an input transform");
+  SATCV_CHECK(!(mode_in && d->in_scale), "igemm: s2d source cannot carry an input transform");
   a.x0 = d->x0; a.x1 = d->x1; a.c0 = d->c0; a.c1 = d->c1;
   a.in_scale = d->in_scale; a.in_shift = d->in_shift; a.in_relu = d->in_relu;
   a.w = d->w; a.bias = d->bias; a.out_scale = d->out_scale; a.y = d->y; a.ldy = d->ldy;
@@ -285,14 +287,14 @@
               "igemm: fused max-pool needs pool_f >= 2 dividing h and w_, plain output mode, whole 16-byte channel vectors");
   a.stats = d->stats; a.stats_ld = d->stats_ld;
   a.n = d->n; a.h = d->h; a.w_ = d->w_;
-  a.hs = d->mode_in ? d->h * d->f : d->h; a.ws = d->mode_in ? d->w_ * d->f : d->w_;
+  a.hs = mode_in ? d->h * d->f : d->h; a.ws = mode_in ? d->w_ * d->f : d->w_;
   a.cout = d->cout; a.cout_pad = d->cout_pad;
   a.kh = d->kh; a.kw = d->kw; a.dil = d->dil;
-  a.mode_in = d->mode_in; a.mode_out = d->mode_out; a.f = d->f;
+  a.mode_in = mode_in; a.mode_out = d->mode_out; a.f = d->f;
   a.cstat = d->cstat; a.out_relu = d->out_relu; a.accumulate = d->accumulate;
   a.stride = d->stride > 1 ? d->stride : 1;
   if (a.stride > 1) {
-    SATCV_CHECK(!d->mode_in && !d->mode_out && d->hin > 0 && d->win > 0 && d->h == (d->hin - 1) / a.stride + 1 && d->w_ == (d->win - 1) / a.stride + 1,
+    SATCV_CHECK(!mode_in && !d->mode_out && d->hin > 0 && d->win > 0 && d->h == (d->hin - 1) / a.stride + 1 && d->w_ == (d->win - 1) / a.stride + 1,
                 "igemm: strided conv needs hin/win with h=(hin-1)/stride+1");
     a.hs = d->hin; a.ws = d->win;
   }
@@ -301,6 +303,13 @@
   a.bst_y = d->bst_y; a.bst_y1 = d->bst_y1; a.bst_ld = d->bst_ld; a.bst_ld1 = d->bst_ld1; a.bst_split = d->bst_y1 ? d->bst_split : 0;
   a.bst_scale = d->bst_scale; a.bst_shift = d->bst_shift; a.bst_mean = d->bst_mean; a.bst_rstd = d->bst_rstd; a.bst_relu = d->bst_relu;
   a.tile_policy = d->tile_policy;
+  a.x0_f32 = nullptr;
+  if (direct) {
+    SATCV_CHECK(d->c0 == 16 && !d->x1 && !d->in_scale && d->dtype == SATCV_BF16 && !d->mode_out && d->stride <= 1,
+                "igemm: mode_in 2 (direct input) needs c0 = 16 presented bf16 channels, one source, no input transform");
+    SATCV_CHECK(((uintptr_t)d->x0 % 16) == 0, "igemm: the direct input must be 16-byte aligned");
+    a.x0_f32 = reinterpret_cast<const float*>(d->x0); a.x0 = nullptr;
+  }
   a.pair_n = d->pair_n; a.pair_c0 = d->pair_c0; a.pair_c1 = d->pair_c1;
   if (d->pair_n || d->pair_c0 || d->pair_c1) {
     const int epv = d->dtype == SATCV_F32 ? 4 : (d->dtype == SATCV_BF16 ? 8 : 16);
@@ -331,6 +340,7 @@
 extern "C" int satcv_conv2d_igemm_pipelined(const satcv_conv_desc* d) {
   IgemmArgs a;
   if (!d || igemm_fill_args(d, a) != SATCV_OK || igemm_force_generic()) return 0;
+  if (a.x0_f32) return igemm_ws_launch(a, d->dtype, nullptr, true) == SATCV_OK ? 1 : 0;
   if (a.kh == 3 && a.kw == 3 && a.stride == 1 && a.dil >= a.h && a.dil >= a.w_) { a.kh = a.kw = 1; a.dil = 1; }
   if (d->bst_y && a.dil == 3) {
     IgemmArgs b = a;
@@ -346,6 +356,13 @@
   if (rc) return rc;
   hipStream_t st = reinterpret_cast<hipStream_t>(stream);
   const double flops = 2.0 * d->n * d->h * d->w_ * (double)d->cout * (double)(a.c0 + a.c1) * d->kh * d->kw;
+  if (a.x0_f32) {
+    satcv_prof_begin(0, flops, st);
+    rc = igemm_ws_launch(a, d->dtype, st, false);
+    satcv_prof_end(0, st);
+    if (rc == SATCV_ERR_UNSUPPORTED) satcv_set_error("igemm: mode_in 2 (direct input) is outside the weights-stationary kernel's limits (ask satcv_conv2d_igemm_pipelined first)");
+    return rc;
+  }
   if (a.kh == 3 && a.kw == 3 && a.stride == 1 && a.dil >= a.h && a.dil >= a.w_) {
     const size_t esz = d->dtype == SATCV_BF16 ? 2 : 4;
     a.w = reinterpret_cast<const unsigned char*>(a.w) + (size_t)4 * ((a.c0 + a.c1) / 8) * a.cout_pad * 8 * esz;
diff --git a/satellite_computervision_amd/csrc/conv_igemm_ws.hip b/satellite_computervision_amd/csrc/conv_igemm_ws.hip
--- a/satellite_computervision_amd/csrc/conv_igemm_ws.hip
+++ b/satellite_computervision_amd/csrc/conv_igemm_ws.hip
@@ -1,6 +1,7 @@
 #include "igemm_common.hpp"
 #include <cstdlib>
 extern int g_opt_igemm_thin;
+extern int g_opt_direct_input;
 int g_ws_launches = 0;
 
 #ifndef SATCV_ABLATE
@@ -14,7 +15,7 @@
 #define STAMP_V(t) do { __builtin_amdgcn_sched_barrier(0); asm volatile("s_waitcnt vmcnt(0)\n\ts_memtime %0\n\ts_waitcnt lgkmcnt(0)" : "=s"(t) :: "memory"); __builtin_amdgcn_sched_barrier(0); } while (0)
 #endif
 
-template <typename T, int CIN, int NT, int WPS, int WN = 1, int DIL = 1>
+template <typename T, int CIN, int NT, int WPS, int WN = 1, int DIL = 1, bool F32SRC = false>
 __global__ __launch_bounds__(256 * WN, WPS) void igemm_ws_kernel(const IgemmArgs a, const int total_tiles) {
   constexpr int TW = 32, TH = 8, WM = 4, MT = 2, BM = 256, BN = WN * NT * 32, NTHREADS = 256 * WN, EL = 8;
   constexpr int SLOTS = CIN / EL, CL = TW + 2 * DIL, PITCH = CL, RL = TH + 2 * DIL;
@@ -43,10 +44,12 @@
     const Raw8<T> v = gload8<T>(wp + ((size_t)run * a.cout_pad + co) * EL);
     lstore8<T>(ldsW + (size_t)it * EL, v);
   }
+  static_assert(!F32SRC || (std::is_same<T, bf16>::value && CIN == 16), "the fp32 source is the 4-channel model input of a 16-channel bf16 layer");
   const int ch0 = slot_t * EL;
-  const bool second = ch0 >= a.c0;
-  const T* src = second ? reinterpret_cast<const T*>(a.x1) + (ch0 - a.c0) : reinterpret_cast<const T*>(a.x0) + ch0;
-  const int cs = second ? a.c1 : a.c0;
+  const bool second = !F32SRC && ch0 >= a.c0;
+  const T* src = F32SRC ? reinterpret_cast<const T*>(a.x0_f32)
+                        : (second ? reinterpret_cast<const T*>(a.x1) + (ch0 - a.c0) : reinterpret_cast<const T*>(a.x0) + ch0);
+  const int cs = F32SRC ? 8 : (second ? a.c1 : a.c0);
   float sc[8], sh[8];
 #pragma unroll
   for (int e = 0; e < 8; ++e) { sc[e] = a.in_scale ? a.in_scale[ch0 + e] : 1.f; sh[e] = a.in_scale ? a.in_shift[ch0 + e] : 0.f; }
@@ -87,7 +90,7 @@
 #pragma unroll
     for (int j = 0; j < AI; ++j) {
       const int dy = a_yx[j] >> 16, dx = (int)(short)(a_yx[j] & 0xffff);
-      const bool ok = a_l[j] >= 0 && dy >= ylo && dy < yhi && dx >= xlo && dx < xhi;
+      const bool ok = a_l[j] >= 0 && dy >= ylo && dy < yhi && dx >= xlo && dx < xhi && (!F32SRC || slot_t == 0);
       vm |= (ok ? 1u : 0u) << j;
       int off = ok ? a_eoff[j] : 0;
       asm volatile("" : "+v"(off));
@@ -118,6 +121,7 @@
 #pragma unroll
     for (int j = 0; j < AI; ++j) {
       Raw8<T> v = ra[j];
+      if constexpr (F32SRC) v = f32x4_to_bf16_item(v);
       if (aff) { if constexpr (std::is_same<T, bf16>::value) v = affine8_lim(v, sc, sh, relu_lim); else v = affine8<T>(v, sc, sh, a.in_relu); }
       v = select8<T>((valid >> j) & 1u, v);
       if (a_l[j] >= 0) lstore8<T>(ldsA + a_l[j], v);
@@ -193,7 +197,7 @@
 #endif
 }
 
-template <typename T, int CIN, int NT, int WPS, int WN = 1, int DIL = 1>
+template <typename T, int CIN, int NT, int WPS, int WN = 1, int DIL = 1, bool F32SRC = false>
 static int ws_cfg(IgemmArgs& a, hipStream_t st, bool dry) {
   constexpr int TW = 32, TH = 8, BN = WN * NT * 32, SLOTS = CIN / 8, RL = TH + 2 * DIL, PITCH = TW + 2 * DIL;
   constexpr int ES = (int)sizeof(T);
@@ -211,7 +215,7 @@
   const long long total = (long long)a.n * a.tiles_y * a.tiles_x;
   if (total <= 0 || total > 0x7fffffffLL) return SATCV_ERR_UNSUPPORTED;
   if (dry) return SATCV_OK;
-  auto kern = igemm_ws_kernel<T, CIN, NT, WPS, WN, DIL>;
+  auto kern = igemm_ws_kernel<T, CIN, NT, WPS, WN, DIL, F32SRC>;
   { const int rc = satcv_ensure_dynamic_lds(reinterpret_cast<const void*>(kern), LDS); if (rc) return rc; }
   static int ncu = 0;
   if (!ncu) {
@@ -234,6 +238,7 @@
 int igemm_ws_launch(IgemmArgs& a, int dtype, hipStream_t st, bool dry) {
   if (!g_opt_igemm_thin || (dtype != SATCV_BF16 && dtype != SATCV_FP8)) return SATCV_ERR_UNSUPPORTED;
   const int cin = a.c0 + a.c1;
+  if (a.x0_f32 && (!g_opt_direct_input || dtype != SATCV_BF16 || cin != 16 || a.x1 || a.in_scale || a.dil != 1 || a.cout != 32 || a.accumulate)) return SATCV_ERR_UNSUPPORTED;
   if (a.kh != 3 || a.kw != 3 || (a.dil != 1 && a.dil != 3) || a.stride != 1 || a.mode_in || a.mode_out || a.bst_y) return SATCV_ERR_UNSUPPORTED;
   if (a.accumulate && (a.accumulate != 1 || dtype != SATCV_BF16 || a.stats || a.pool_y || a.out_relu || a.out_scale)) return SATCV_ERR_UNSUPPORTED;
   if (a.pool_y && (8 % a.pool_f != 0 || 32 % a.pool_f != 0)) return SATCV_ERR_UNSUPPORTED;
@@ -257,7 +262,7 @@
     return cin == 32 ? ws_cfg<fp8, 32, 2, 2>(a, st, dry) : ws_cfg<fp8, 64, 1, 1, 2>(a, st, dry);
   }
   if (a.cout == 32) {
-    if (cin == 16) return ws_cfg<bf16, 16, 1, 3>(a, st, dry);
+    if (cin == 16) return a.x0_f32 ? ws_cfg<bf16, 16, 1, 3, 1, 1, true>(a, st, dry) : ws_cfg<bf16, 16, 1, 3>(a, st, dry);
     if (cin == 32) return ws_cfg<bf16, 32, 1, 3>(a, st, dry);
     return ws_cfg<bf16, 64, 1, 2>(a, st, dry);
   }
diff --git a/satellite_computervision_amd/csrc/elementwise.hip b/satellite_computervision_amd/csrc/elementwise.hip
--- a/satellite_computervision_amd/csrc/elementwise.hip
+++ b/satellite_computervision_amd/csrc/elementwise.hip
@@ -121,7 +121,9 @@
   }
 }
 template <typename T>
-__global__ __launch_bounds__(EW_BLOCK) void pack_batched_kernel(const satcv_pack_job* __restrict__ jobs, const long long* __restrict__ prefix, int njobs, long long total) {
+__global__ __launch_bounds__(EW_BLOCK) void pack_batched_kernel(const satcv_pack_job* __restrict__ jobs, const long long* __restrict__ prefix, int njobs, long long total,
+                                                                float* __restrict__ adam_state) {
+  if (adam_state && blockIdx.x == 0 && threadIdx.x == 0) adam_state[1] += 1.f;
   for (long long g0 = (long long)blockIdx.x * EW_BLOCK; g0 < total; g0 += (long long)gridDim.x * EW_BLOCK) {
     int lo = 0, hi = njobs - 1;
     while (lo < hi) { const int mid = (lo + hi + 1) >> 1; if (prefix[mid] <= g0) lo = mid; else hi = mid - 1; }
@@ -160,14 +162,18 @@
   const int64_t real = (int64_t)(j->mode >= 2 ? 1 : j->taps) * (j->kpad / 8) * j->npad;
   return (real + EW_BLOCK - 1) / EW_BLOCK * EW_BLOCK;
 }
-extern "C" int satcv_pack_weights_batched(const satcv_pack_job* jobs_dev, const int64_t* prefix_dev, int32_t njobs, int64_t total_items, int32_t dtype,
-                                          void* stream) {
+extern "C" int satcv_pack_weights_batched_bump(const satcv_pack_job* jobs_dev, const int64_t* prefix_dev, int32_t njobs, int64_t total_items, int32_t dtype,
+                                               float* adam_state, void* stream) {
   SATCV_CHECK(jobs_dev && prefix_dev && njobs > 0 && total_items > 0, "pack_weights_batched: bad args");
   SATCV_CHECK(total_items % EW_BLOCK == 0, "pack_weights_batched: the prefix table must be built from satcv_pack_job_items (multiples of 256)");
   DISPATCH_T8(dtype, hipLaunchKernelGGL(pack_batched_kernel<T>, dim3(ew_grid(total_items)), dim3(EW_BLOCK), 0, (hipStream_t)stream, jobs_dev,
-                                        (const long long*)prefix_dev, njobs, (long long)total_items));
+                                        (const long long*)prefix_dev, njobs, (long long)total_items, adam_state));
   LAUNCH_OK("pack_weights_batched");
   return SATCV_OK;
+}
+extern "C" int satcv_pack_weights_batched(const satcv_pack_job* jobs_dev, const int64_t* prefix_dev, int32_t njobs, int64_t total_items, int32_t dtype,
+                                          void* stream) {
+  return satcv_pack_weights_batched_bump(jobs_dev, prefix_dev, njobs, total_items, dtype, nullptr, stream);
 }
 
 extern "C" int satcv_pack_weights(const float* src, void* dst_fwd, void* dst_dgrad, int32_t kh, int32_t kw, int32_t cin, int32_t cout, int32_t cin_pad, int32_t transposed, int32_t dtype, void* stream) {
@@ -1674,7 +1680,8 @@
 }
 extern "C" int satcv_zero2(void* a, int64_t bytes_a, void* b, int64_t bytes_b, void* stream) {
   SATCV_CHECK(bytes_a >= 0 && bytes_b >= 0 && (bytes_a == 0 || a) && (bytes_b == 0 || b), "zero2: bad args");
-  SATCV_CHECK(((uintptr_t)a % 16 == 0) && bytes_a % 16 == 0 && ((uintptr_t)b % 4 == 0) && bytes_b % 4 == 0, "zero2: a must be 16-byte, b 4-byte aligned and sized");
+  SATCV_CHECK((bytes_a == 0 || (uintptr_t)a % 16 == 0) && bytes_a % 16 == 0 && (bytes_b == 0 || (uintptr_t)b % 4 == 0) && bytes_b % 4 == 0,
+              "zero2: a must be 16-byte, b 4-byte aligned and sized");
   if (bytes_a == 0 && bytes_b == 0) return SATCV_OK;
   hipLaunchKernelGGL(zero2_kernel, dim3(ew_grid(bytes_a / 16 + 1, 4096)), dim3(256), 0, (hipStream_t)stream, reinterpret_cast<uint4*>(a), (long long)(bytes_a / 16),
                      reinterpret_cast<unsigned*>(b), (long long)(bytes_b / 4));
diff --git a/satellite_computervision_amd/csrc/igemm_common.hpp b/satellite_computervision_amd/csrc/igemm_common.hpp
--- a/satellite_computervision_amd/csrc/igemm_common.hpp
+++ b/satellite_computervision_amd/csrc/igemm_common.hpp
@@ -27,6 +27,7 @@
   int ksplit; float* kslab;
   int tile_policy;
   int pair_n, pair_c0, pair_c1;
+  const float* x0_f32;
 };
 
 template <typename T>
diff --git a/satellite_computervision_amd/engine.py b/satellite_computervision_amd/engine.py
--- a/satellite_computervision_amd/engine.py
+++ b/satellite_computervision_amd/engine.py
@@ -86,6 +86,21 @@
     @property
     def c(self):
         return sum(c for _, c in self.srcs)
+
+
+class _LazySrcs(list):
+
+    def __init__(self, srcs, refresh):
+        super().__init__(srcs)
+        self._refresh = refresh
+
+    def __iter__(self):
+        self._refresh()
+        return super().__iter__()
+
+    def __getitem__(self, i):
+        self._refresh()
+        return super().__getitem__(i)
 
 
 def _fp(t, off=0):
@@ -211,17 +226,25 @@
         pre = torch.tensor(prefix, dtype=torch.int64, device=self.dev)
         return dict(jobs=raw, prefix=pre, n=len(jobs), total=tot)
 
-    def repack(self, lo=0, hi=None, stream=None):
+    def _ptab(self, lo, hi):
         if not self.packed:
-            return
+            return None
         key = (lo, hi)
         if key not in self._ptabs:
             self._ptabs[key] = self._pack_table(lo, hi)
-        t = self._ptabs[key]
+        return self._ptabs[key]
+
+    def repack_launches(self, lo=0, hi=None):
+        return self._ptab(lo, hi) is not None
+
+    def repack(self, lo=0, hi=None, stream=None, bump=False):
+        t = self._ptab(lo, hi)
         if t is None:
+            if bump:
+                raise RuntimeError('repack(bump=True) without a launch: ask repack_launches() first')
             return
-        check(lib.satcv_pack_weights_batched(t['jobs'].data_ptr(), t['prefix'].data_ptr(), t['n'], t['total'], self.dtype,
-                                             ops.stream_ptr() if stream is None else stream))
+        check(lib.satcv_pack_weights_batched_bump(t['jobs'].data_ptr(), t['prefix'].data_ptr(), t['n'], t['total'], self.dtype,
+                                                  self.adam_state.data_ptr() if bump else None, ops.stream_ptr() if stream is None else stream))
 
     def ensure_adam(self):
         if self.adam_m is None:
@@ -251,6 +274,8 @@
         self.x_inputs = []
         self.x_by_tid = {}
         self.x_src = {}
+        self._direct_cand = {}
+        self.direct_inputs = set()
         _sp = os.environ.get('SATCV_SIDE_PRIORITY')
         self.side = (torch.cuda.Stream(priority=int(_sp)) if _sp is not None else torch.cuda.Stream()) if (training and rt.model.wgrad_side_stream) else None
         self.step_count = 0
@@ -259,6 +284,7 @@
         self.amax_of = {}
         self._bn_jobs = []
         self._build()
+        self._bind_direct_inputs()
         if self._bn_jobs:
             tab = torch.tensor([[int(v or 0) for v in j] for j in self._bn_jobs], dtype=torch.int64).to(rt.dev)
             self.keep.append(tab)
@@ -281,6 +307,7 @@
         d = ops.make_conv_desc(**kw)
         self.keep.append(d)
         fn = lambda st, d=d: check(lib.satcv_conv2d_igemm(C.byref(d), st))
+        fn.desc = d
         k, cin, cout = kw.get('kh', 1) * kw.get('kw', 1), kw.get('c0', 0) + (kw.get('c1', 0) or 0), kw['cout']
         px = kw['n'] * kw['h'] * kw['w_']
         fn.label = (f"conv_{role} k{kw.get('kh', 1)} d{kw.get('dil', 1)} n{kw['n']} {kw['h']}x{kw['w_']} {kw.get('c0', 0)}+{kw.get('c1', 0) or 0}->{cout}"
@@ -349,6 +376,27 @@
             st_ptr, ld, self.n, hh, ww, c, f, dt, st)))
         return TRef([(act, c)], self.n, hh, ww) if actslot is None else None
 
+    def _bind_direct_inputs(self):
+        for tid, c in self._direct_cand.items():
+            fd, bd = c['fwd'], c['bwd']
+            if fd is None or bd is None:
+                continue
+            x0 = (fd.x0, bd.x0)
+            fd.x0, fd.mode_in = c['xin'].data_ptr(), 2
+            bd.x0, bd.x0_f32, bd.x0_c = None, c['xin'].data_ptr(), 4
+            nb = lib.satcv_conv2d_bwd_fused_workspace(C.byref(bd))
+            if lib.satcv_conv2d_igemm_pipelined(C.byref(fd)) != 1 or nb < 0 or nb > c['bwd_ws']:
+                fd.x0, fd.mode_in = x0[0], 0
+                bd.x0, bd.x0_f32, bd.x0_c = x0[1], None, 0
+                continue
+
+            def bind(st, fd=fd, bd=bd, xin=c['xin'], tid=tid):
+                fd.x0 = bd.x0_f32 = self.x_src.get(tid) or xin.data_ptr()
+            bind.label = 'direct input: the first layer reads the fp32 batch (no ingest launch)'
+            self.fwd[self.fwd.index(c['ingest'])] = bind
+            self.direct_inputs.add(tid)
+            self.vals[tid].srcs = _LazySrcs(self.vals[tid].srcs, lambda ing=c['ingest']: ing(ops.stream_ptr()))
+
     def _build(self):
         rt, m, n = self.rt, self.rt.model, self.n
         T, dt, es = rt.tdtype, rt.dtype, rt.esize
@@ -413,8 +461,12 @@
                 self.x_by_tid[t.id] = xin
                 npix = n * self.h * self.w
                 cc = t.channels
-                self.fwd.append(lambda st, xin=xin, x=x, npix=npix, cc=cc, cp=cp, tid=t.id: check(lib.satcv_ingest_nhwc(
-                    self.x_src.get(tid) or xin.data_ptr(), x.data_ptr(), npix, cc, cp, dt, st)))
+                ing = lambda st, xin=xin, x=x, npix=npix, cc=cc, cp=cp, tid=t.id: check(lib.satcv_ingest_nhwc(
+                    self.x_src.get(tid) or xin.data_ptr(), x.data_ptr(), npix, cc, cp, dt, st))
+                ing.label = f'ingest_nhwc n{n} {self.h}x{self.w} {cc}->{cp}'
+                self.fwd.append(ing)
+                if training and dt == BF16 and cc == 4 and len(consumers[t.id]) == 1 and consumers[t.id][0].op == 'cba':
+                    self._direct_cand[t.id] = dict(xin=xin, ingest=ing, fwd=None, bwd=None)
                 vals[t.id] = TRef([(x, cp)], n, self.h, self.w)
             elif op == 'cba':
                 tin, tout = node.inputs[0], node.outputs[0]
@@ -486,6 +538,8 @@
                                                 stats=_fp(stats, aoff), stats_ld=ldy, n=n, h=r.h, w_=r.w, cout=cout, cout_pad=rup(cout, 32),
                                                 kh=k, kw=k, dil=dil, dtype=dt, stride=stride, hin=hin if stride > 1 else 0,
                                                 win=win if stride > 1 else 0, **self._src_args(r)))
+                if tin.id in self._direct_cand and stride == 1:
+                    self._direct_cand[tin.id]['fwd'] = self.fwd[-1].desc
                 aff = self._bn_forward(lay.bn_name, stats, ldy, aoff, cout, n * r.h * r.w, node.attrs.get('bn_updates', 1), aff_in, aoff)
                 if sl is None:
                     vals[tout.id] = TRef([(y, cout)], n, r.h, r.w, affine=aff, relu=relu_out)
@@ -1178,6 +1232,8 @@
                         fused_ws_need = max(fused_ws_need, nbp)
                     fdescs.append(fzp)
                     self.keep.append(fzp)
+                    if not want_dx and tin.id in self._direct_cand:
+                        self._direct_cand[tin.id].update(bwd=fzp, bwd_ws=nbp)
                     self.bwd += [fin] if (pre is not None or red is None) else [red, fin]
                     fstep = lambda st, fzp=fzp: check(lib.satcv_conv2d_bwd_fused(C.byref(fzp), st))
                     fstep.label = f"bwd_fused k3 n{n} {hh}x{ww} {sa['c0']}+{sa['c1']}->{cout} pooled{'' if want_dx else ' nodx'}{' +poolsums' if fzp.bst_sums else ''}"
diff --git a/satellite_computervision_amd/model_tools.py b/satellite_computervision_amd/model_tools.py
--- a/satellite_computervision_amd/model_tools.py
+++ b/satellite_computervision_amd/model_tools.py
@@ -1137,17 +1137,12 @@
         plan.run_backward(st)
         if sync_grads is not None:
             sync_grads(rt.gflat)
-        if plan.eo_done:
-            lo = plan.eo_lo
-            check(lib.satcv_adam_step_part(rt.pflat.data_ptr(), rt.gflat.data_ptr(), rt.adam_m.data_ptr(), rt.adam_v.data_ptr(), lo,
-                                           opt.beta_1, opt.beta_2, opt.epsilon, rt.adam_state.data_ptr(),
-                                           rt.lr_mul.data_ptr() if rt.lr_mul is not None else None, 1, st))
-            rt.repack(0, lo)
-        else:
-            check(lib.satcv_adam_step(rt.pflat.data_ptr(), rt.gflat.data_ptr(), rt.adam_m.data_ptr(), rt.adam_v.data_ptr(), rt.pflat.numel(),
-                                      opt.beta_1, opt.beta_2, opt.epsilon, rt.adam_state.data_ptr(),
-                                      rt.lr_mul.data_ptr() if rt.lr_mul is not None else None, st))
-            rt.repack()
+        hi = plan.eo_lo if plan.eo_done else rt.pflat.numel()
+        in_pack = rt.repack_launches(0, plan.eo_lo if plan.eo_done else None)
+        check(lib.satcv_adam_step_part(rt.pflat.data_ptr(), rt.gflat.data_ptr(), rt.adam_m.data_ptr(), rt.adam_v.data_ptr(), hi,
+                                       opt.beta_1, opt.beta_2, opt.epsilon, rt.adam_state.data_ptr(),
+                                       rt.lr_mul.data_ptr() if rt.lr_mul is not None else None, 0 if in_pack else 1, st))
+        rt.repack(0, plan.eo_lo if plan.eo_done else None, bump=in_pack)
         self._weights_version = getattr(self, '_weights_version', 0) + 1
         return plan
 
diff --git a/satellite_computervision_amd/ops.py b/satellite_computervision_amd/ops.py
--- a/satellite_computervision_amd/ops.py
+++ b/satellite_computervision_amd/ops.py
@@ -115,6 +115,19 @@
     return y
 
 
+def conv2d_direct_input(x_f32, w_packed, cout, *, bias=None, stats=None):
+    n, h, w_, c = x_f32.shape
+    if c != 4 or x_f32.dtype != torch.float32 or not x_f32.is_contiguous():
+        return None
+    y = torch.empty(n, h, w_, rup(cout, 16), dtype=torch.bfloat16, device=x_f32.device)
+    d = make_conv_desc(x0=_p(x_f32), c0=16, mode_in=2, w=_p(w_packed), y=_p(y), ldy=y.shape[-1], n=n, h=h, w_=w_, cout=cout, cout_pad=rup(cout, 32),
+                       dtype=BF16, bias=_p(bias), stats=_p(stats), stats_ld=stats.shape[-1] if stats is not None else 0)
+    if lib.satcv_conv2d_igemm_pipelined(C.byref(d)) != 1:
+        return None
+    check(lib.satcv_conv2d_igemm(C.byref(d), stream_ptr()))
+    return y
+
+
 def conv2d_transpose(x, w_packed, cout, f, *, bias=None, in_scale=None, in_shift=None, in_relu=False, stats=None, out=None,
                      out_scale=None, out_relu=False):
     n, h, w_, c0 = x.shape
@@ -169,9 +182,10 @@
 def make_bwdf_desc(*, g, yraw, ldg, bn_scale, bn_shift, bn_mean, bn_rstd, bn_coef, x0, c0, w_dgrad, dx, lddx, dw, cin, cout, n, h, w_, dtype,
                    linear=0, x1=None, c1=0, in_scale=None, in_shift=None, in_relu=0, kh=3, kw=3, dil=1, workspace=None, workspace_bytes=0,
                    accumulate=0, bst_sums=None, bst_sums_ld=0, bst_mean=None, bst_rstd=None, bst_act_form=0, dpool=None, lddp=0, amax=None,
-                   hg_dlogits=None, hg_w=None, hg_ncls=0):
+                   hg_dlogits=None, hg_w=None, hg_ncls=0, x0_f32=None, x0_c=0):
     from ._lib import BwdfDesc
     d = BwdfDesc()
+    d.x0_f32, d.x0_c = x0_f32, int(x0_c)
     d.g, d.yraw, d.ldg = g, yraw, ldg
     d.bn_scale, d.bn_shift, d.bn_mean, d.bn_rstd, d.bn_coef, d.linear = bn_scale, bn_shift, bn_mean, bn_rstd, bn_coef, int(linear)
     d.x0, d.x1, d.c0, d.c1 = x0, x1, c0, c1
@@ -186,22 +200,24 @@
 
 
 def conv_bwd_fused(g, yraw, scale, shift, mean, rstd, coef, x, w_dgrad, cin, cout, *, x1=None, in_scale=None, in_shift=None, in_relu=False,
-                   linear=False, accumulate_into=None, bst=None, dpool=None, amax=None, want_dx=True, head=None):
-    n, h, w_, c0 = x.shape
+                   linear=False, accumulate_into=None, bst=None, dpool=None, amax=None, want_dx=True, head=None, x_f32=None):
+    dev, xdt = (x if x_f32 is None else x_f32).device, (x.dtype if x_f32 is None else torch.bfloat16)
+    n, h, w_, c0 = x.shape if x_f32 is None else tuple(x_f32.shape[:3]) + (16,)
     c1 = x1.shape[-1] if x1 is not None else 0
-    dx = torch.empty(n, h, w_, c0 + c1, dtype=x.dtype, device=x.device) if want_dx else None
-    dw = accumulate_into if accumulate_into is not None else torch.empty(3, 3, cin, cout, dtype=torch.float32, device=x.device)
+    dx = torch.empty(n, h, w_, c0 + c1, dtype=xdt, device=dev) if want_dx else None
+    dw = accumulate_into if accumulate_into is not None else torch.empty(3, 3, cin, cout, dtype=torch.float32, device=dev)
     d = make_bwdf_desc(g=_p(g), yraw=_p(yraw), ldg=g.shape[-1] if g is not None else yraw.shape[-1], bn_scale=_p(scale), bn_shift=_p(shift), bn_mean=_p(mean), bn_rstd=_p(rstd),
                        bn_coef=_p(coef), x0=_p(x), c0=c0, x1=_p(x1), c1=c1, in_scale=_p(in_scale), in_shift=_p(in_shift), in_relu=in_relu,
-                       w_dgrad=_p(w_dgrad), dx=_p(dx), lddx=c0 + c1, dw=_p(dw), cin=cin, cout=cout, n=n, h=h, w_=w_, dtype=DTYPE_CODE[x.dtype],
+                       w_dgrad=_p(w_dgrad), dx=_p(dx), lddx=c0 + c1, dw=_p(dw), cin=cin, cout=cout, n=n, h=h, w_=w_, dtype=DTYPE_CODE[xdt],
                        linear=linear, accumulate=accumulate_into is not None, dpool=_p(dpool), lddp=dpool.shape[-1] if dpool is not None else 0,
-                       amax=_p(amax), **(dict(hg_dlogits=_p(head[0]), hg_w=_p(head[1]), hg_ncls=head[0].shape[-1]) if head else {}),
+                       amax=_p(amax), **(dict(x0_f32=_p(x_f32), x0_c=x_f32.shape[-1]) if x_f32 is not None else {}),
+                       **(dict(hg_dlogits=_p(head[0]), hg_w=_p(head[1]), hg_ncls=head[0].shape[-1]) if head else {}),
                        **(dict(bst_sums=_p(bst['sums']), bst_sums_ld=bst['sums'].shape[-1], bst_mean=_p(bst.get('mean')), bst_rstd=_p(bst.get('rstd')),
                                bst_act_form=bst.get('act_form', 0)) if bst else {}))
     nb = lib.satcv_conv2d_bwd_fused_workspace(C.byref(d))
     if nb < 0:
         return None
-    ws = torch.empty(max(nb // 4, 1), dtype=torch.float32, device=x.device)
+    ws = torch.empty(max(nb // 4, 1), dtype=torch.float32, device=dev)
     d.workspace, d.workspace_bytes = ws.data_ptr(), nb
     check(lib.satcv_conv2d_bwd_fused(C.byref(d), stream_ptr()))
     return dx, dw
```

New measurement: 8304 tiles/s (median of 6 runs). No clear change (+0.8%).
